# QizhiPei/FABind

Measured on AMD Instinct MI355X. Metric: complexes/sec fwd+bwd (1500p/40l nodes), full IaBNet on the whole graph (pocket model + 4-layer complex model + distance-map head on all nodes / pairs) with the pocket-cls + pocket-centre + coord + distmap + distmap-by-coords + distill losses (BASELINE configs[2] read literally), higher is better.
Workload: dtype bf16

## Files before the change

### fabind_amd/_lib.py

```python
import ctypes
import os

import torch

from . import config as _cfg

_HERE = os.path.dirname(os.path.abspath(__file__))
LIB_PATH = _cfg.knob("FABIND_LIB") or os.path.join(_HERE, "libfabind_hip.so")

ABI_VERSION = 19
DT_F32, DT_BF16 = 0, 1
ACT_NONE, ACT_SILU, ACT_RELU, ACT_SIGMOID, ACT_STORED_DERIV = 0, 1, 2, 3, 4
GEMM_FAM_NT_F32, GEMM_FAM_NT_F32_BF16, GEMM_FAM_NT_BF16, GEMM_FAM_GLDS, GEMM_FAM_PIPE, GEMM_FAM_X3, GEMM_FAM_X3_PRO, GEMM_FAM_PERSIST = range(8)

LNR_8S16, LNR_8S32, LNR_V8_1, LNR_V8_2, LNR_V8_3, LNR_V8_4, LNR_S2, LNR_S8, LNR_S16, LNR_S32, LNR_COUNT = range(11)
LNB_8S16, LNB_8S32, LNB_V8_1, LNB_V8_2, LNB_V8_3, LNB_S2, LNB_S8, LNB_S16, LNB_S20, LNB_S32, LNB_COUNT = range(11)
RST_BF16_1, RST_BF16_2, RST_BF16_4, RST_GENERIC, RST_COUNT = range(5)
ELF_WAVE1, ELF_WAVE1_TAIL, ELF_WAVE2_TAIL, ELF_CHUNK, ELF_COUNT = range(5)
ELB_NPL1, ELB_NPL2, ELB_NPL3, ELB_COUNT = range(4)

_vp, _i, _f, _l = ctypes.c_void_p, ctypes.c_int, ctypes.c_float, ctypes.c_long


class GemmArgs(ctypes.Structure):
# ... 58 lines not shown
    "fabind_gcl_edge_fused_bwd_set_tile": [_i],
    "fabind_gcl_edge_fused_bwd_tile": [],
    "fabind_gcl_edge_fused_bwd_set_variant": [_i],
    "fabind_gcl_edge_fused_set_variant": [_i],
    "fabind_gcl_edge_fused_variant": [],
    "fabind_gcl_edge_fused_bwd_variant": [],
    "fabind_gcl_edge_fused_bwd_variant_for": [_i],
    "fabind_row_stats": [_vp, _i, _i, _f, _i, _i, _vp, _vp, _vp],
    "fabind_layernorm_rows": [_vp, _i, _i, _vp, _vp, _f, _i, _i, _vp, _i, _i, _i, _vp],
    "fabind_edge_ln_concat": [_vp, _i, _i, _vp, _vp, _vp, _vp, _vp, _f, _i, _vp, _i, _i, _i, _vp],
    "fabind_edge_lnfold": [_vp, _i, _i, _i, _vp, _vp, _vp, _vp, _f, _vp, _vp, _vp, _vp, _i, _vp, _f, ctypes.c_uint, _vp],
    "fabind_edge_lnfold_bwd_blocks": [_i],
    "fabind_edge_lnfold_bwd": [_vp, _i, _i, _i, _vp, _vp, _vp, _vp, _f, _vp, _vp, _vp, _vp, _vp, _i, _f, _vp, _vp, _vp, _vp, _i, _vp],
    "fabind_layernorm_rows_form": [_vp, _i, _i, _vp, _i, _i],
    "fabind_layernorm_rows_bwd_form": [_vp, _i, _vp, _i, _vp, _i, _i],
    "fabind_row_stats_form": [_vp, _i, _i, _i],
    "fabind_edge_lnfold_form": [_i, _i, ctypes.POINTER(_i)],
    "fabind_edge_lnfold_blocks": [_i],
    "fabind_edge_lnfold_bwd_form": [_i, ctypes.POINTER(_i)],
    "fabind_inter_coord_fold_blocks": [_i],
    "fabind_inter_coord_fold": [_vp, _i, _i, _vp, _vp, _vp, _f, _f, _vp, _vp, _vp, _i, _vp, _f, ctypes.c_uint, _vp],
    "fabind_post_optimize": [_vp, _vp, _vp, _vp, _vp, _i, _i, _i, _i, _f, _vp, _vp, _vp, _vp],
    "fabind_distmap_generate": [_vp, _vp, _vp, _vp, _vp, _vp, _vp, _vp, _vp, _vp, _i, _i, _i, _i, _i, _i, _l, _i, _i, _i, _i,
                                _vp, _vp, _vp, _vp, _vp, _vp, _vp, _vp],
    "fabind_sym_automorphisms": [_vp, _vp, _vp, _vp, _i, _i, _i, _vp, _vp, _vp, _vp, _vp, _vp],
    "fabind_sym_score": [_vp, _i, _i, _vp, _vp, _vp, _vp, _vp, _i, _i, _vp, _vp, _vp, _vp, _vp, _vp],
    "fabind_pose_stats": [_vp, _vp, _vp, _i, _vp, _vp, _vp],
    "fabind_rank_loss_fwd": [_vp, _vp, _vp, _i, _i, _i, _vp, _vp, _vp, _vp],
    "fabind_multi_copy": [_vp, _i, _i, _vp],
    "fabind_adam_chunk": [],
    "fabind_multi_sqnorm": [_vp, _i, _i, _vp, _vp, _vp, _vp],
    "fabind_multi_adam": [_vp, _i, _i, _vp, _vp, _vp, _f, _i, _vp, _vp, _vp],
    "fabind_zero_empty_rows": [_vp, _i, _vp, _i, _i, _i, _vp, _i, _i, _vp],
    "fabind_split_sum": [_vp, _i, ctypes.c_long, _vp, _i, ctypes.c_long, _vp, _vp],
    "fabind_segment_sum": [_vp, _i, _i, _i, _vp, _vp, _i, _i, _i, _vp, _i, _vp, _i, _vp],
    "fabind_coord_update": [_vp, _vp, _vp, _i, _vp, _vp, _i, _i, _f, _vp, _vp, _vp],
    "fabind_cross_attn_fwd": [_vp, _i, _vp, _vp, _i, _vp, _i, _vp, _i, _i, _i, _vp, _i, _i, _f, _vp, _i, _vp, _i, _vp, _i,
                              _vp],
    "fabind_cross_attn_mfma_fwd": [_vp, _i, _vp, _vp, _i, _vp, _i, _vp, _i, _i, _i, _vp, _i, _i, _f, _vp, _i, _vp, _i, _vp, _i,
                                   _vp],
    "fabind_cross_attn_fused_fwd": [_vp, _i, _vp, _vp, _i, _vp, _i, _vp, _i, _vp, _vp, _vp, _vp, _i, _i, _i, _i, _i, _f, _vp, _i, _vp, _i, _vp, _vp],
    "fabind_cross_attn_fused_bwd": [ctypes.POINTER(AttnFusedBwdArgs), _i, _i, _i, _i, _i, _i, _vp],
    "fabind_pair_bot_pack": [_vp, _i, _vp, _i, _vp, _vp, _vp, _vp, _i, _vp, _i, _l, _vp],
    "fabind_pair_bo_pack": [_vp, _i, _vp, _i, _vp, _vp, _vp, _vp, _i, _vp, _i, _l, _vp],
    "fabind_cross_attn_mfma_bwd": [_vp, _i, _vp, _i, _vp, _i, _i, _i, _vp, _i, _i, _i, _f, _vp, _vp, _vp, _vp, _vp, _vp, _vp,
                                   _vp, _vp, _vp],
    "fabind_pair_bmat": [_vp, _i, _vp, _i, _i, _vp, _i, _vp, _i, _vp],
    "fabind_pair_hadamard": [_vp, _vp, _i, _i, _vp, _vp, _i, _i, _vp, _vp, _i, _vp, _i, _i, _vp],
    "fabind_inter_attn_fwd": [_vp, _i, _vp, _i, _i, _vp, _i, _vp, _vp, _vp, _vp, _vp, _vp, _vp, _i, _vp, _vp, _vp,
                              _vp, _f, _i, _vp, _vp, _vp, _vp, _vp, _vp, _vp],
    "fabind_inter_attn_fwd_rows": [_vp, _i, _vp, _i, _i, _vp, _i, _vp, _vp, _vp, _vp, _vp, _vp, _vp, _i, _vp, _vp, _vp,
                                   _vp, _f, _i, _vp, _vp, _vp, _vp, _vp, _vp, _vp, _i, _i, _vp],
    "fabind_layernorm_rows_bwd": [_vp, _i, _i, _vp, _vp, _i, _i, _f, _i, _i, _vp, _i, _i, _vp, _vp, _i, _vp],
    "fabind_edge_concat": [_vp, _i, _i, _vp, _vp, _vp, _i, _vp, _i, _i, _i, _vp],
    "fabind_las_step": [_vp, _vp, _vp, _vp, _vp, _vp, _vp, _i, _i, _f, _f, _vp, _vp, _vp],
    "fabind_select_rows": [_vp, _vp, _vp, _i, _i, _vp, _vp],
    "fabind_add": [_vp, _vp, _vp, _l, _vp],
    "fabind_mul_dact": [_vp, _i, _vp, _i, _i, _vp, _i, _l, _f, _vp],
    "fabind_mul_dact_colsum": [_vp, _i, _vp, _i, _i, _vp, _i, _i, _i, _vp, _vp, _i, _f, _vp],
    "fabind_drop_mix": [_vp, _vp, _vp, _l, _f, ctypes.c_uint, _vp],
    "fabind_drop_mix_bwd": [_vp, _vp, _vp, _l, _f, ctypes.c_uint, _vp],
    "fabind_mul_dropmask_colsum": [_vp, _i, _vp, _i, _i, _i, _f, ctypes.c_uint, _vp, _vp, _i, _vp],
    "fabind_rowdot_bwd": [_vp, _i, _vp, _i, _vp, _i, _i, _i, _vp, _vp, _vp, _i, _vp],
    "fabind_edge_geom_bwd": [_vp, _vp, _vp, _vp, _vp, _vp, _vp, _vp, _vp, _vp, _i, _i, _i, _vp, _vp, _vp, _vp],
    "fabind_gcl_pre_bwd": [_vp, _i, _i, _vp, _vp, _i, _vp, _vp, _vp, _i, _vp],
    "fabind_gather_dact": [_vp, _i, _vp, _vp, _i, _i, _vp, _i, _i, _i, _vp],
    "fabind_coord_update_bwd": [_vp, _vp, _vp, _i, _i, _f, _vp, _vp, _vp, _vp],
    "fabind_cross_attn_bwd": [_vp, _i, _vp, _i, _vp, _i, _i, _i, _vp, _i, _i, _i, _f, _vp, _vp, _vp, _vp, _vp, _vp, _vp,
                              _vp, _vp, _vp],
    "fabind_pair_bias_cat": [_vp, _i, _vp, _i, _i, _i, _vp, _i, _vp, _i, _vp, _vp, _i, _vp, _i, _vp, _vp],
    "fabind_batched_transpose_pad": [_vp, _i, _vp, _i, _i, _i, _i, _vp, _vp],
    "fabind_node_chain_fwd": [_vp, _i, _vp, _i, _vp, _vp, _vp, _vp, _vp, _vp, _i, _i, _vp, _i, _vp, _i, _vp, _i, _i, _i, _vp],
    "fabind_node_chain_x3_fwd": [_vp, _i, _vp, _i, _vp, _vp, _vp, _vp, _vp, _vp, _vp, _vp, _vp, _vp, _i, _i, _vp, _i, _vp, _i, _vp, _i, _vp, _i, _vp, _i,
                                 _i, _i, _vp],
    "fabind_rows_hadamard_bwd": [_vp, _i, _i, _vp, _i, _i, _vp, _vp, _vp, _i, _vp, _i, _vp],
    "fabind_pair_hadamard_bwd_grid": [_vp, _i, _i, _vp, _i, _i, _vp, _vp, _vp, _vp, _i, _vp, _i, _vp],
    "fabind_pair_hadamard_bwd_rows": [_vp, _i, _i, _vp, _i, _i, _vp, _i, _i, _vp, _vp, _vp, _vp, _i, _vp, _i, _vp, _i, _vp],
    "fabind_pair_hadamard_bwd": [_vp, _i, _i, _vp, _vp, _i, _i, _vp, _vp, _i, _i, _vp, _vp, _i, _vp, _vp, _i, _vp, _vp, _i,
                                 _vp],
    "fabind_inter_attn_bwd": [_vp, _i, _vp, _i, _i, _vp, _vp, _vp, _vp, _vp, _vp, _vp, _vp, _vp, _vp, _vp, _vp, _f, _i,
                              _vp, _vp, _vp, _vp, _vp, _vp, _vp, _vp, _vp, _vp, _i, _vp],
    "fabind_inter_attn_bwd_rows": [_vp, _i, _vp, _i, _i, _vp, _vp, _vp, _vp, _vp, _vp, _vp, _vp, _vp, _vp, _vp, _vp, _f, _i,
                                   _vp, _vp, _vp, _vp, _vp, _vp, _vp, _vp, _vp, _vp, _i, _vp, _i, _i, _vp],
    "fabind_las_step_bwd": [_vp, _vp, _vp, _vp, _vp, _vp, _vp, _vp, _i, _i, _f, _f, _vp, _vp, _vp],
    "fabind_pair_bias_bwd": [_vp, _i, _vp, _i, _i, _vp, _vp, _i, _i, _i, _vp, _vp, _vp, _vp, _vp],
    "fabind_pair_bias_btcat": [_vp, _i, _vp, _vp, _vp, _i, _i, _i, _vp, _i, _i, _vp],
    "fabind_pair_bias_finish": [_vp, _vp, _i, _i, _vp, _vp, _i, _vp, _vp, _l, _vp],
    "fabind_pack_frag_multi": [_vp, _vp, _i, _vp],
    "fabind_lower_bound": [_vp, _i, _vp, _i, _vp, _vp],
    "fabind_pocket_center_fwd": [_vp, _vp, _vp, _vp, _i, _i, _f, _i, _vp, _vp, _vp],
    "fabind_pocket_center_bwd": [_vp, _vp, _vp, _vp, _i, _i, _f, _vp, _vp, _vp, _vp, _vp],
    "fabind_pair_dist_fwd": [_vp, _i, _i, _vp, _vp, _f, _f, _f, _vp, _vp],
    "fabind_pair_dist_bwd": [_vp, _i, _i, _vp, _vp, _vp, _f, _f, _f, _vp, _vp, _vp],
    "fabind_block_hadamard_fwd": [_vp, _i, _i, _vp, _i, _vp, _i, _i, _vp, _i, _vp],
    "fabind_block_hadamard_bwd": [_vp, _i, _i, _vp, _i, _vp, _i, _vp, _i, _i, _vp, _i, _i, _vp, _vp, _i, _vp, _i, _vp],
    "fabind_loss_fwd": [_vp, _vp, _l, _vp, _vp, _vp, _l, _vp, _vp, _i, _vp, _l, _vp, _vp, _l, _f, _f, _f, _f, _f, _f, _vp, _vp, _vp, _vp, _vp, _vp],
    "fabind_loss_bwd": [_vp, _vp, _l, _vp, _vp, _vp, _l, _vp, _vp, _i, _l, _vp, _vp, _l, _f, _f, _f, _f, _f, _f, _vp, _vp, _vp,
                        _vp, _vp, _vp, _vp, _vp, _vp],
    "fabind_layernorm_fwd": [_vp, _vp, _vp, _f, _i, _i, _vp, _vp, _vp, _vp],
    "fabind_layernorm_bwd": [_vp, _vp, _vp, _vp, _vp, _i, _i, _vp, _vp, _vp, _vp],
}

_lib = None


def load():
    global _lib
    if _lib is not None:
        return _lib
    if not os.path.exists(LIB_PATH):
        raise RuntimeError(
            "fabind_amd: %s is missing -- build it with `python -m fabind_amd.build` (hipcc, gfx950). "
            "There is no CPU/eager fallback for the hot path." % LIB_PATH)
    lib = ctypes.CDLL(LIB_PATH)
    lib.fabind_last_error.restype = ctypes.c_char_p
    lib.fabind_abi_version.restype = ctypes.c_int
    got = lib.fabind_abi_version()
    if got != ABI_VERSION:
        raise RuntimeError("fabind_amd: %s has ABI version %d, this binding needs %d -- rebuild with `python -m fabind_amd.build`"
                           % (LIB_PATH, got, ABI_VERSION))
    lib.fabind_sizeof_args.argtypes, lib.fabind_sizeof_args.restype = [ctypes.c_int], ctypes.c_int
    lib.fabind_cross_attn_bwd_scratch.argtypes, lib.fabind_cross_attn_bwd_scratch.restype = [_i, _i, _i], ctypes.c_long
    lib.fabind_pair_bias_cat_parts.argtypes, lib.fabind_pair_bias_cat_parts.restype = [_i, _i], ctypes.c_long
    lib.fabind_cross_attn_fused_bwd_scratch.argtypes, lib.fabind_cross_attn_fused_bwd_scratch.restype = [_i, _i, _i, _i, _i], ctypes.c_long
    lib.fabind_cross_attn_fused_bwd_parts.argtypes, lib.fabind_cross_attn_fused_bwd_parts.restype = [_i, _i], ctypes.c_int
    lib.fabind_pair_bias_finish_parts.argtypes, lib.fabind_pair_bias_finish_parts.restype = [_i], ctypes.c_int
    lib.fabind_loss_blocks.argtypes, lib.fabind_loss_blocks.restype = [_l, _l, _l], ctypes.c_int
    for nm in ("fabind_pair_block_tile", "fabind_pair_block_chunk"):
        getattr(lib, nm).argtypes, getattr(lib, nm).restype = [], ctypes.c_int
    for which, mirror in enumerate((GemmArgs, EdgeBwdArgs, PairUpdateArgs, TnJob, AttnFusedBwdArgs, AdamRow)):
        if lib.fabind_sizeof_args(which) != ctypes.sizeof(mirror):
            raise RuntimeError("fabind_amd: ctypes mirror %s is %d bytes, the library's struct is %d -- _lib.py and "
                               "include/fabind_hip.h disagree" % (mirror.__name__, ctypes.sizeof(mirror),
                                                                  lib.fabind_sizeof_args(which)))
    for nm in ("fabind_gemm_set_config", "fabind_gemm_set_persistent", "fabind_gemm_set_small_m", "fabind_gemm_set_x3_tile", "fabind_gemm_tn_set_waves",
               "fabind_gemm_tn_set_exp", "fabind_gcl_edge_fused_set_xcd_aware", "fabind_gcl_edge_fused_bwd3_set_exp",
               "fabind_gcl_edge_fused_bwd4_set_exp"):
        getattr(lib, nm).argtypes, getattr(lib, nm).restype = [ctypes.c_int], None
    lib.fabind_gemm_tn_tile_n.argtypes, lib.fabind_gemm_tn_tile_n.restype = [], ctypes.c_int
    for name, argt in SIGNATURES.items():
        fn = getattr(lib, name)
        fn.argtypes = argt
        fn.restype = ctypes.c_int
    for k in _cfg.KNOBS.values():
        if k.category == "native-dev" and _cfg.knob(k.name) is not None:
            getattr(lib, k.setter)(_cfg.knob(k.name))
    _lib = lib
    return lib


_DEBUG_SYNC = _cfg.knob("FABIND_DEBUG_SYNC")


def check(rc, what):
    if rc != 0:
        raise RuntimeError("%s failed (rc=%d): %s" % (what, rc, load().fabind_last_error().decode()))
    if _DEBUG_SYNC:
        print("[fabind] " + what, flush=True)
        torch.cuda.synchronize()


def ptr(t):
    if t is None:
        return None
    if not t.is_cuda:
        raise RuntimeError("fabind_amd kernels need HIP device tensors; got a %s tensor" % t.device)
# ... 20 lines not shown
```

### fabind_amd/csrc/gcl.hip

```cpp
#include "common.h"
#include "fabind_hip.h"

__global__ __launch_bounds__(256) void gcl_pre_kernel(const void* __restrict__ AB, int ab_dt, int ldab, int H,
                                                      const int* row, const int* col, const float* rhohat,
                                                      const float* __restrict__ w_r, void* pre, int pre_dt, int E, int act,
                                                      void* dact_out) {
    const int lane = threadIdx.x & 63;
    int e = blockIdx.x * 4 + (threadIdx.x >> 6);
    if (e >= E) return;
    const size_t a = (size_t)row[e] * ldab, b = (size_t)col[e] * ldab + H;
    const float rh = rhohat[e];
    for (int c = lane * 4; c < H; c += 256) {
        float4 va = ld4_any(AB, ab_dt, a + c), vb = ld4_any(AB, ab_dt, b + c), w = *(const float4*)(w_r + c);
        const float4 z = make_float4(va.x + vb.x + rh * w.x, va.y + vb.y + rh * w.y, va.z + vb.z + rh * w.z,
                                     va.w + vb.w + rh * w.w);
        st4_any(pre, pre_dt, (size_t)e * H + c,
                make_float4(apply_act(z.x, act), apply_act(z.y, act), apply_act(z.z, act), apply_act(z.w, act)));
        if (dact_out)
            st4_any(dact_out, pre_dt, (size_t)e * H + c,
                    make_float4(apply_dact(z.x, act), apply_dact(z.y, act), apply_dact(z.z, act), apply_dact(z.w, act)));
    }
}

#define GP_PASSES 4
// ... 79 lines not shown
                      (!dact_out || (uintptr_t)dact_out % 16 == 0) && ((uintptr_t)w_r % 16 == 0);
#define GP_LAUNCH4(LPE_, A16_, O16_, D_)                                                                             \
    hipLaunchKernelGGL((gcl_pre8_kernel<LPE_, A16_, O16_, D_>),                                                      \
                       dim3((E + 4 * (64 / LPE_) * GP_PASSES - 1) / (4 * (64 / LPE_) * GP_PASSES)), dim3(256), 0, stream, \
                       AB, ldab, row, col, rhohat, w_r, pre, E, act, dact_out)
#define GP_LAUNCH(LPE_)                                                                                              \
    do {                                                                                                             \
        const bool a16 = ab_dt == FB_DT_BF16, o16 = pre_dt == FB_DT_BF16;                                            \
        if (a16 && o16 && dact_out) GP_LAUNCH4(LPE_, true, true, true);                                              \
        else if (a16 && o16) GP_LAUNCH4(LPE_, true, true, false);                                                    \
        else if (!a16 && o16 && dact_out) GP_LAUNCH4(LPE_, false, true, true);                                       \
        else if (!a16 && o16) GP_LAUNCH4(LPE_, false, true, false);                                                  \
        else if (!a16 && !o16 && dact_out) GP_LAUNCH4(LPE_, false, false, true);                                     \
        else if (!a16 && !o16) GP_LAUNCH4(LPE_, false, false, false);                                                \
        else if (dact_out) GP_LAUNCH4(LPE_, true, false, true);                                                      \
        else GP_LAUNCH4(LPE_, true, false, false);                                                                   \
    } while (0)
    if (vec8 && H == 512) GP_LAUNCH(64);
    else if (vec8 && H == 256) GP_LAUNCH(32);
    else if (vec8 && H == 128) GP_LAUNCH(16);
    else if (vec8 && H == 64) GP_LAUNCH(8);
    else
        hipLaunchKernelGGL(gcl_pre_kernel, dim3((E + 3) / 4), dim3(256), 0, stream, AB, ab_dt, ldab, H, row, col, rhohat,
                           w_r, pre, pre_dt, E, act, dact_out);
#undef GP_LAUNCH
#undef GP_LAUNCH4
    FB_CHECK_LAUNCH();
    return 0;
}


template <int NSLAB, int U>
__device__ __forceinline__ void ss_accum(const void* __restrict__ Z, int z_dt, int ldz, int H, const int* eidx, int act,
                                         int lane, int e0, int e1, int estep, F8 (&acc)[NSLAB]) {
    int ee = e0;
    for (; ee + (U - 1) * estep < e1; ee += U * estep) {
        int e[U];
#pragma unroll
        for (int u = 0; u < U; ++u) e[u] = eidx ? eidx[ee + u * estep] : ee + u * estep;
#pragma unroll
        for (int s = 0; s < NSLAB; ++s) {
            const int c = s * 512 + lane * 8;
            if (c < H) {
                F8 v[U];
#pragma unroll
                for (int u = 0; u < U; ++u) v[u] = ld8_any(Z, z_dt, (size_t)e[u] * ldz + c);
#pragma unroll
                for (int u = 0; u < U; ++u)
#pragma unroll
                    for (int k = 0; k < 8; ++k) acc[s].v[k] += apply_act(v[u].v[k], act);
            }
        }
    }
    if (ee < e1) {
        int e[U];
        bool ok[U];
#pragma unroll
        for (int u = 0; u < U; ++u) {
            ok[u] = ee + u * estep < e1;
            e[u] = ok[u] ? (eidx ? eidx[ee + u * estep] : ee + u * estep) : 0;
        }
#pragma unroll
        for (int s = 0; s < NSLAB; ++s) {
            const int c = s * 512 + lane * 8;
            if (c < H) {
                F8 v[U];
#pragma unroll
                for (int u = 0; u < U; ++u) {
                    if (ok[u]) v[u] = ld8_any(Z, z_dt, (size_t)e[u] * ldz + c);
                    else
#pragma unroll
                        for (int k = 0; k < 8; ++k) v[u].v[k] = 0.f;
                }
#pragma unroll
                for (int u = 0; u < U; ++u)
#pragma unroll
                    for (int k = 0; k < 8; ++k) acc[s].v[k] += apply_act(v[u].v[k], act);
            }
        }
    }
}

template <int NSLAB>
__global__ __launch_bounds__(256) void segment_sum_kernel(const void* __restrict__ Z, int z_dt, int ldz, int H,
                                                          const int* rowptr, const int* eidx, int act, float* out,
                                                          int ldo, int n_rows, bf16_t* out16, int ldo16, int heavy_min) {
    const int lane = threadIdx.x & 63;
    const int r = blockIdx.x * 4 + (threadIdx.x >> 6);
    if (r >= n_rows) return;
    const int e0 = rowptr[r], e1 = rowptr[r + 1];
    if (e1 - e0 > heavy_min) return;
    F8 acc[NSLAB];
#pragma unroll
    for (int s = 0; s < NSLAB; ++s)
#pragma unroll
        for (int k = 0; k < 8; ++k) acc[s].v[k] = 0.f;
    ss_accum<NSLAB, 8 / NSLAB>(Z, z_dt, ldz, H, eidx, act, lane, e0, e1, 1, acc);
#pragma unroll
    for (int s = 0; s < NSLAB; ++s) {
        const int c = s * 512 + lane * 8;
        if (c < H) {
            if (out) {
                float* o = out + (size_t)r * ldo + c;
                *(float4*)o = make_float4(acc[s].v[0], acc[s].v[1], acc[s].v[2], acc[s].v[3]);
                *(float4*)(o + 4) = make_float4(acc[s].v[4], acc[s].v[5], acc[s].v[6], acc[s].v[7]);
            }
            if (out16) st8_any(out16, FB_DT_BF16, (size_t)r * ldo16 + c, acc[s]);
        }
    }
}

template <int NSLAB>
__global__ __launch_bounds__(1024) void segment_sum_heavy_kernel(const void* __restrict__ Z, int z_dt, int ldz, int H,
                                                                 const int* rowptr, const int* eidx, int act, float* out,
                                                                 int ldo, int n_rows, bf16_t* out16, int ldo16, int rpw, int heavy_min) {
    __shared__ F8 part[15][NSLAB * 64];
    __shared__ int heavy[1024];
    __shared__ int n_heavy;
    const int lane = threadIdx.x & 63, w = threadIdx.x >> 6;
    if (threadIdx.x == 0) n_heavy = 0;
    __syncthreads();
    const int rr = blockIdx.x * rpw + threadIdx.x;
    if ((int)threadIdx.x < rpw && rr < n_rows && rowptr[rr + 1] - rowptr[rr] > heavy_min) heavy[atomicAdd(&n_heavy, 1)] = rr;
    __syncthreads();
    const int nh = n_heavy;
    for (int q = 0; q < nh; ++q) {
        const int r = heavy[q];
        F8 acc[NSLAB];
#pragma unroll
        for (int s = 0; s < NSLAB; ++s)
#pragma unroll
            for (int k = 0; k < 8; ++k) acc[s].v[k] = 0.f;
        ss_accum<NSLAB, 8 / NSLAB>(Z, z_dt, ldz, H, eidx, act, lane, rowptr[r] + w, rowptr[r + 1], 16, acc);
        if (w > 0) {
#pragma unroll
            for (int s = 0; s < NSLAB; ++s) part[w - 1][s * 64 + lane] = acc[s];
        }
        __syncthreads();
        if (w == 0) {
#pragma unroll
            for (int s = 0; s < NSLAB; ++s) {
                for (int k = 0; k < 15; ++k) {
                    const F8 p = part[k][s * 64 + lane];
#pragma unroll
                    for (int t = 0; t < 8; ++t) acc[s].v[t] += p.v[t];
                }
                const int c = s * 512 + lane * 8;
                if (c < H) {
                    if (out) {
                        float* o = out + (size_t)r * ldo + c;
                        *(float4*)o = make_float4(acc[s].v[0], acc[s].v[1], acc[s].v[2], acc[s].v[3]);
                        *(float4*)(o + 4) = make_float4(acc[s].v[4], acc[s].v[5], acc[s].v[6], acc[s].v[7]);
                    }
                    if (out16) st8_any(out16, FB_DT_BF16, (size_t)r * ldo16 + c, acc[s]);
                }
            }
        }
        __syncthreads();
    }
}

extern "C" int fabind_segment_sum(const void* Z, int z_dt, int ldz, int H, const int* rowptr, const int* eidx,
                                  int n_rows, int n_edges, int act, float* out, int ldo, void* out16v, int ldo16,
                                  hipStream_t stream) {
    bf16_t* out16 = (bf16_t*)out16v;
    FB_REQUIRE(H % 8 == 0 && ldz % 8 == 0 && ldo % 4 == 0, "fabind_segment_sum: H/ldz must be multiples of 8, ldo of 4");
    FB_REQUIRE(H <= 1024, "fabind_segment_sum: H <= 1024");
    FB_REQUIRE(out != nullptr || out16 != nullptr, "fabind_segment_sum: no output");
    FB_REQUIRE(((uintptr_t)Z % 16 == 0) && ((uintptr_t)out % 16 == 0), "fabind_segment_sum: 16-byte alignment");
    FB_REQUIRE(out16 == nullptr || (ldo16 % 8 == 0 && (uintptr_t)out16 % 16 == 0), "fabind_segment_sum: out16 needs 16-byte alignment and ldo16 % 8 == 0");
    if (n_rows <= 0) return 0;
    (void)n_edges;
    int rpw = 1024;
    while (rpw > 64 && (n_rows + rpw - 1) / rpw < 256) rpw >>= 1;
    const int heavy_min = n_rows < 16384 ? 32 : 128;
    const dim3 g((n_rows + 3) / 4), gh((n_rows + rpw - 1) / rpw);
    if (H <= 512) {
        hipLaunchKernelGGL((segment_sum_kernel<1>), g, dim3(256), 0, stream, Z, z_dt, ldz, H, rowptr, eidx, act, out, ldo, n_rows, out16, ldo16, heavy_min);
        hipLaunchKernelGGL((segment_sum_heavy_kernel<1>), gh, dim3(1024), 0, stream, Z, z_dt, ldz, H, rowptr, eidx, act, out, ldo, n_rows, out16, ldo16, rpw, heavy_min);
    } else {
        hipLaunchKernelGGL((segment_sum_kernel<2>), g, dim3(256), 0, stream, Z, z_dt, ldz, H, rowptr, eidx, act, out, ldo, n_rows, out16, ldo16, heavy_min);
        hipLaunchKernelGGL((segment_sum_heavy_kernel<2>), gh, dim3(1024), 0, stream, Z, z_dt, ldz, H, rowptr, eidx, act, out, ldo, n_rows, out16, ldo16, rpw, heavy_min);
    }
    FB_CHECK_LAUNCH();
    return 0;
}

__global__ __launch_bounds__(256) void coord_update_kernel(const float* __restrict__ x, const float* __restrict__ d,
                                                           const float* __restrict__ s_part, int n_part,
                                                           const float* weight, const int* rowptr, int n_rows, int mean,
                                                           float clampv, float* x_out, float* s_out) {
    const int lane = threadIdx.x & 63;
    int r = blockIdx.x * 4 + (threadIdx.x >> 6);
    if (r >= n_rows) return;
    const int e0 = rowptr[r], e1 = rowptr[r + 1];
    float ax = 0.f, ay = 0.f, az = 0.f;
    for (int e = e0 + lane; e < e1; e += 64) {
        float s = 0.f;
        for (int k = 0; k < n_part; ++k) s += s_part[(size_t)e * n_part + k];
        if (weight) s *= weight[e];
        if (s_out) s_out[e] = s;
        ax += d[(size_t)e * 3] * s; ay += d[(size_t)e * 3 + 1] * s; az += d[(size_t)e * 3 + 2] * s;
    }
    ax = wave_sum(ax); ay = wave_sum(ay); az = wave_sum(az);
    if (lane == 0) {
        const int deg = e1 - e0;
        const float den = mean ? (float)(deg < 1 ? 1 : deg) : 1.f;
        float tx = ax / den, ty = ay / den, tz = az / den;
        tx = fminf(fmaxf(tx, -clampv), clampv); ty = fminf(fmaxf(ty, -clampv), clampv); tz = fminf(fmaxf(tz, -clampv), clampv);
        x_out[(size_t)r * 3] = x[(size_t)r * 3] + tx;
        x_out[(size_t)r * 3 + 1] = x[(size_t)r * 3 + 1] + ty;
        x_out[(size_t)r * 3 + 2] = x[(size_t)r * 3 + 2] + tz;
    }
}

extern "C" int fabind_coord_update(const float* x, const float* d, const float* s_part, int n_part,
                                   const float* weight, const int* rowptr, int n_rows, int mean, float clampv,
                                   float* x_out, float* s_out, hipStream_t stream) {
    if (n_rows <= 0) return 0;
    hipLaunchKernelGGL(coord_update_kernel, dim3((n_rows + 3) / 4), dim3(256), 0, stream, x, d, s_part, n_part, weight,
                       rowptr, n_rows, mean, clampv, x_out, s_out);
    FB_CHECK_LAUNCH();
    return 0;
}

__global__ __launch_bounds__(256) void zero_empty_rows_kernel(const int* __restrict__ rowptr, int n_rows, void* out, int out_dt, int ld,
                                                              int C, void* out2, int out2_dt, int ld2) {
    const int lane = threadIdx.x & 63;
    const int r = blockIdx.x * 4 + (threadIdx.x >> 6);
    if (r >= n_rows || rowptr[r] != rowptr[r + 1]) return;
    for (int c = lane; c < C; c += 64) {
        st_any(out, out_dt, (size_t)r * ld + c, 0.f);
        if (out2) st_any(out2, out2_dt, (size_t)r * ld2 + c, 0.f);
    }
}

extern "C" int fabind_zero_empty_rows(const int* rowptr, int n_rows, void* out, int out_dt, int ld, int C, void* out2, int out2_dt,
                                      int ld2, hipStream_t stream) {
    if (n_rows <= 0 || C <= 0) return 0;
    FB_REQUIRE(rowptr != nullptr && out != nullptr, "fabind_zero_empty_rows: rowptr / out");
    hipLaunchKernelGGL(zero_empty_rows_kernel, dim3((n_rows + 3) / 4), dim3(256), 0, stream, rowptr, n_rows, out, out_dt, ld, C, out2,
                       out2_dt, ld2);
    FB_CHECK_LAUNCH();
    return 0;
}


__global__ __launch_bounds__(256) void pack_frag_multi_kernel(const FabindPackSeg* __restrict__ segs) {
    const FabindPackSeg sg = segs[blockIdx.y];
    const int N = sg.N, Kd = sg.K;
    const long n_vec = (long)N * Kd / 8;
    bf16_t* dst = (bf16_t*)sg.dst;
    for (long t = (long)blockIdx.x * 256 + threadIdx.x; t < n_vec; t += (long)gridDim.x * 256) {
        const int r = (int)(t & 15), q = (int)((t >> 4) & 3);
        const long tb = t >> 6;
        const int nb = (int)(tb % (N / 16)), kb = (int)(tb / (N / 16));
        const long n = (long)nb * 16 + r, k0 = (long)kb * 32 + q * 8;
        uint32_t w[4];
#pragma unroll
        for (int j = 0; j < 4; ++j) {
            float a, b;
            const long i0 = n * sg.src_sr + (k0 + 2 * j) * sg.src_sc, i1 = i0 + sg.src_sc;
            if (sg.src_dt == FB_DT_BF16) {
                a = bf16_to_f32(((const bf16_t*)sg.src)[i0]);
                b = bf16_to_f32(((const bf16_t*)sg.src)[i1]);
            } else {
// ... 30 lines not shown
```

### fabind_amd/csrc/inter_attn_rows.hip

```cpp
#include "common.h"
#include "fabind_hip.h"

#define IA_HEAVY 8

template <int NS>
__global__ __launch_bounds__(256) void inter_attn_fwd_rows_kernel(
    const float* __restrict__ qkv, int ldqkv, const float* __restrict__ cv, int ldcv, int H, const float* __restrict__ h,
    int ldh, const float* __restrict__ x, const float* __restrict__ d, const float* __restrict__ rhohat,
    const int* rowptr, const int* col, const int* red_idx, const float* bias_red, int bias_np,
    const float* __restrict__ w_rk, const float* __restrict__ w_rv, const float* __restrict__ wcr,
    const float* __restrict__ w3, float clampv, int n_rows, float* h_out, float* x_out, float* alpha, float* cvs, bf16_t* h16,
    const float* __restrict__ s_ext, const int* __restrict__ order, int n_heavy, int n_act) {
    __shared__ float4 sAcc[4][NS * 64];
    __shared__ float sSc[4][8];
    const int lane = threadIdx.x & 63, wv = threadIdx.x >> 6;
    const bool coop = (int)blockIdx.x < n_heavy;
    const int idx = coop ? (int)blockIdx.x : n_heavy + ((int)blockIdx.x - n_heavy) * 4 + wv;
    if (idx >= n_rows) return;
    const int r = order[idx];
    if (idx >= n_act) {
#pragma unroll
        for (int s = 0; s < NS; ++s) {
            const int c = s * 256 + lane * 4;
            if (c < H) {
// ... 98 lines not shown
        for (int s = 0; s < NS; ++s) {
            const int c = s * 256 + lane * 4;
            if (c < H) {
                const float4 hv = *(const float4*)(h + (size_t)r * ldh + c);
                const float4 wvv = *(const float4*)(w_rv + c);
                const float4 o = make_float4(hv.x + (acc[s].x + sar * wvv.x) * inv, hv.y + (acc[s].y + sar * wvv.y) * inv,
                                             hv.z + (acc[s].z + sar * wvv.z) * inv, hv.w + (acc[s].w + sar * wvv.w) * inv);
                *(float4*)(h_out + (size_t)r * ldh + c) = o;
                if (h16) *(uint2*)(h16 + (size_t)r * H + c) = make_uint2(pack2_bf16(o.x, o.y), pack2_bf16(o.z, o.w));
            }
        }
        if (lane == 0) {
            const float tx = fminf(fmaxf(ax * inv, -clampv), clampv), ty = fminf(fmaxf(ay * inv, -clampv), clampv),
                        tz = fminf(fmaxf(az * inv, -clampv), clampv);
            x_out[(size_t)r * 3] = x[(size_t)r * 3] + tx;
            x_out[(size_t)r * 3 + 1] = x[(size_t)r * 3 + 1] + ty;
            x_out[(size_t)r * 3 + 2] = x[(size_t)r * 3 + 2] + tz;
        }
    } else {
#pragma unroll
        for (int s = 0; s < NS; ++s) sAcc[wv][s * 64 + lane] = acc[s];
        if (lane == 0) { sSc[wv][0] = m; sSc[wv][1] = l; sSc[wv][2] = sar; sSc[wv][3] = ax; sSc[wv][4] = ay; sSc[wv][5] = az; }
        __syncthreads();
        const float M = fmaxf(fmaxf(sSc[0][0], sSc[1][0]), fmaxf(sSc[2][0], sSc[3][0]));
        float f[4], L = 0.f, SAR = 0.f, AX = 0.f, AY = 0.f, AZ = 0.f;
#pragma unroll
        for (int w = 0; w < 4; ++w) {
            f[w] = sSc[w][1] > 0.f ? __expf(sSc[w][0] - M) : 0.f;
            L += f[w] * sSc[w][1]; SAR += f[w] * sSc[w][2]; AX += f[w] * sSc[w][3]; AY += f[w] * sSc[w][4]; AZ += f[w] * sSc[w][5];
        }
        inv = 1.f / L;
        for (int g = threadIdx.x; g < NS * 64; g += 256) {
            const int c = (g >> 6) * 256 + (g & 63) * 4;
            if (c < H) {
                float4 a = make_float4(0.f, 0.f, 0.f, 0.f);
#pragma unroll
                for (int w = 0; w < 4; ++w) {
                    const float4 p = sAcc[w][g];
                    a.x += f[w] * p.x; a.y += f[w] * p.y; a.z += f[w] * p.z; a.w += f[w] * p.w;
                }
                const float4 hv = *(const float4*)(h + (size_t)r * ldh + c);
                const float4 wvv = *(const float4*)(w_rv + c);
                const float4 o = make_float4(hv.x + (a.x + SAR * wvv.x) * inv, hv.y + (a.y + SAR * wvv.y) * inv,
                                             hv.z + (a.z + SAR * wvv.z) * inv, hv.w + (a.w + SAR * wvv.w) * inv);
                *(float4*)(h_out + (size_t)r * ldh + c) = o;
                if (h16) *(uint2*)(h16 + (size_t)r * H + c) = make_uint2(pack2_bf16(o.x, o.y), pack2_bf16(o.z, o.w));
            }
        }
        if (threadIdx.x == 0) {
            const float tx = fminf(fmaxf(AX * inv, -clampv), clampv), ty = fminf(fmaxf(AY * inv, -clampv), clampv),
                        tz = fminf(fmaxf(AZ * inv, -clampv), clampv);
            x_out[(size_t)r * 3] = x[(size_t)r * 3] + tx;
            x_out[(size_t)r * 3 + 1] = x[(size_t)r * 3 + 1] + ty;
            x_out[(size_t)r * 3 + 2] = x[(size_t)r * 3 + 2] + tz;
        }
        m = M;
    }
    __builtin_amdgcn_fence(__ATOMIC_RELEASE, "wavefront");
    __builtin_amdgcn_fence(__ATOMIC_ACQUIRE, "wavefront");
    for (int e = ws + lane; e < we; e += 64) alpha[e] = __expf(alpha[e] - m) * inv;
}

extern "C" int fabind_inter_attn_fwd_rows(const float* qkv, int ldqkv, const float* cv, int ldcv, int H, const float* h,
                                          int ldh, const float* x, const float* d, const float* rhohat, const int* rowptr,
                                          const int* col, const int* red_idx, const float* bias_red, int bias_np,
                                          const float* w_rk, const float* w_rv, const float* wcr, const float* w3,
                                          float clampv, int n_rows, float* h_out, float* x_out, float* alpha, float* cvs,
                                          const float* s_ext, void* h16, const int* order, int n_heavy, int n_act, hipStream_t stream) {
    FB_REQUIRE(H % 4 == 0 && ldqkv % 4 == 0 && ldcv % 4 == 0 && ldh % 4 == 0, "fabind_inter_attn_fwd_rows: % 4");
    FB_REQUIRE(H <= 1024, "fabind_inter_attn_fwd_rows: H <= 1024");
    FB_REQUIRE(order != nullptr && 0 <= n_heavy && n_heavy <= n_act && n_act <= n_rows, "fabind_inter_attn_fwd_rows: order / counts");
    if (n_rows <= 0) return 0;
    dim3 grid(n_heavy + (n_rows - n_heavy + 3) / 4), block(256);
#define LAUNCH(NS)                                                                                                   \
    hipLaunchKernelGGL((inter_attn_fwd_rows_kernel<NS>), grid, block, 0, stream, qkv, ldqkv, cv, ldcv, H, h, ldh, x, d, \
                       rhohat, rowptr, col, red_idx, bias_red, bias_np, w_rk, w_rv, wcr, w3, clampv, n_rows, h_out, \
                       x_out, alpha, cvs, (bf16_t*)h16, s_ext, order, n_heavy, n_act)
    if (H <= 256) LAUNCH(1); else if (H <= 512) LAUNCH(2); else LAUNCH(4);
#undef LAUNCH
    FB_CHECK_LAUNCH();
    return 0;
}

template <int NS>
__global__ __launch_bounds__(256) void inter_attn_bwd_a_rows_kernel(
    const float* __restrict__ qkv, int ldqkv, const float* __restrict__ cv, int ldcv, int H, const float* __restrict__ d,
    const float* __restrict__ rhohat, const int* rowptr, const int* col, const float* __restrict__ w_rk,
    const float* __restrict__ w_rv, const float* __restrict__ wcr, const float* __restrict__ w3, const float* alpha,
    const float* cvs, float clampv, int n_rows, const float* __restrict__ dh_out, const float* __restrict__ dx_out,
    float* dqkv, float* dd, float* drh, float* dlogit, float* dcp, float* wpart, const int* __restrict__ order, int n_heavy, int n_act) {
    extern __shared__ float4 shp[];
    float (*sS)[4] = (float (*)[4])(shp + 4 * NS * 64);
    const int lane = threadIdx.x & 63, wv = threadIdx.x >> 6;
    const float4 z4 = make_float4(0.f, 0.f, 0.f, 0.f);
    float4 a_wrk[NS], a_wrv[NS], a_wcr[NS], a_w3[NS], wk[NS], wvv[NS], wc[NS], w3v[NS];
#pragma unroll
    for (int s = 0; s < NS; ++s) {
        const int c = s * 256 + lane * 4;
        a_wrk[s] = z4; a_wrv[s] = z4; a_wcr[s] = z4; a_w3[s] = z4; wk[s] = z4; wvv[s] = z4; wc[s] = z4; w3v[s] = z4;
        if (c < H) {
            wk[s] = *(const float4*)(w_rk + c); wvv[s] = *(const float4*)(w_rv + c);
            wc[s] = *(const float4*)(wcr + c); w3v[s] = *(const float4*)(w3 + c);
        }
    }
    const int n_hturns = (n_heavy + (int)gridDim.x - 1) / (int)gridDim.x;
    const int n_lturns = (n_rows - n_heavy + (int)gridDim.x * 4 - 1) / ((int)gridDim.x * 4);
    for (int turn = 0; turn < n_hturns + n_lturns; ++turn) {
        const bool coop = turn < n_hturns;
        int idx;
        if (coop) idx = turn * (int)gridDim.x + (int)blockIdx.x;
        else idx = n_heavy + ((turn - n_hturns) * (int)gridDim.x + (int)blockIdx.x) * 4 + wv;
        if (coop ? idx >= n_heavy : idx >= n_rows) continue;
        const int r = order[idx];
        if (idx >= n_act) {
#pragma unroll
            for (int s = 0; s < NS; ++s) {
                const int c = s * 256 + lane * 4;
                if (c < H) *(float4*)(dqkv + (size_t)r * ldqkv + c) = z4;
            }
            continue;
        }
        const int e0 = rowptr[r], e1 = rowptr[r + 1];
        int ws = e0, we = e1;
        if (coop) {
            const int per = (e1 - e0 + 3) >> 2;
            ws = min(e1, e0 + wv * per);
            we = min(e1, ws + per);
        }
        float4 qv[NS], gh[NS], dq[NS];
        float qw = 0.f, gwv = 0.f;
#pragma unroll
        for (int s = 0; s < NS; ++s) {
            const int c = s * 256 + lane * 4;
            qv[s] = z4; gh[s] = z4; dq[s] = z4;
            if (c < H) {
                qv[s] = *(const float4*)(qkv + (size_t)r * ldqkv + c);
                gh[s] = *(const float4*)(dh_out + (size_t)r * H + c);
                qw += qv[s].x * wk[s].x + qv[s].y * wk[s].y + qv[s].z * wk[s].z + qv[s].w * wk[s].w;
                gwv += gh[s].x * wvv[s].x + gh[s].y * wvv[s].y + gh[s].z * wvv[s].z + gh[s].w * wvv[s].w;
            }
        }
        qw = wave_sum(qw); gwv = wave_sum(gwv);
        float tx = 0.f, ty = 0.f, tz = 0.f;
        for (int e = e0 + lane; e < e1; e += 64) {
            const float w = alpha[e] * cvs[e];
            tx += w * d[(size_t)e * 3]; ty += w * d[(size_t)e * 3 + 1]; tz += w * d[(size_t)e * 3 + 2];
        }
        tx = wave_sum(tx); ty = wave_sum(ty); tz = wave_sum(tz);
        const float gx = fabsf(tx) <= clampv ? dx_out[(size_t)r * 3] : 0.f;
        const float gy = fabsf(ty) <= clampv ? dx_out[(size_t)r * 3 + 1] : 0.f;
        const float gz = fabsf(tz) <= clampv ? dx_out[(size_t)r * 3 + 2] : 0.f;
        float S = 0.f;
        float4 pa[NS], pb[NS];
        auto fetch_v = [&](int cn) {
#pragma unroll
            for (int s = 0; s < NS; ++s) {
                const int c = s * 256 + lane * 4;
                pa[s] = z4;
                if (c < H) pa[s] = *(const float4*)(qkv + (size_t)cn * ldqkv + 2 * H + c);
            }
        };
        for (int eb = ws; eb < we; eb += 64) {
            const int ne = min(64, we - eb);
            int my_col = 0;
            float my_rh = 0.f, my_al = 0.f, my_cvs = 0.f, my_gd = 0.f, my_da = 0.f;
            if (lane < ne) {
                const int e = eb + lane;
                my_col = col[e]; my_rh = rhohat[e]; my_al = alpha[e]; my_cvs = cvs[e];
                my_gd = gx * d[(size_t)e * 3] + gy * d[(size_t)e * 3 + 1] + gz * d[(size_t)e * 3 + 2];
            }
            fetch_v(__shfl(my_col, 0, 64));
            for (int j = 0; j < ne; ++j) {
                const float rh = __shfl(my_rh, j, 64);
                float hp = 0.f;
                float4 vv[NS];
#pragma unroll
                for (int s = 0; s < NS; ++s) vv[s] = pa[s];
                if (j + 1 < ne) fetch_v(__shfl(my_col, j + 1, 64));
#pragma unroll
                for (int s = 0; s < NS; ++s)
                    hp += gh[s].x * vv[s].x + gh[s].y * vv[s].y + gh[s].z * vv[s].z + gh[s].w * vv[s].w;
                hp = wave_sum(hp) + rh * gwv;
                const float da = hp + __shfl(my_cvs, j, 64) * __shfl(my_gd, j, 64);
                S += __shfl(my_al, j, 64) * da;
                if (lane == j) my_da = da;
            }
            if (lane < ne) dlogit[eb + lane] = my_da;
        }
        if (coop) {
            if (lane == 0) sS[wv][0] = S;
            __syncthreads();
            S = ((sS[0][0] + sS[1][0]) + sS[2][0]) + sS[3][0];
        }
        __builtin_amdgcn_fence(__ATOMIC_RELEASE, "wavefront");
        __builtin_amdgcn_fence(__ATOMIC_ACQUIRE, "wavefront");
        float s_lrh = 0.f, s_arh = 0.f;
        auto fetch_kc = [&](int cn) {
#pragma unroll
            for (int s = 0; s < NS; ++s) {
                const int c = s * 256 + lane * 4;
                pa[s] = z4; pb[s] = z4;
                if (c < H) {
                    pa[s] = *(const float4*)(qkv + (size_t)cn * ldqkv + H + c);
                    pb[s] = *(const float4*)(cv + (size_t)cn * ldcv + c);
                }
            }
        };
        for (int eb = ws; eb < we; eb += 64) {
            const int ne = min(64, we - eb);
            int my_col = 0;
            float my_rh = 0.f, my_al = 0.f, my_cvs = 0.f, my_gd = 0.f, my_da = 0.f, o_dl = 0.f, o_dc = 0.f, o_drh = 0.f;
            if (lane < ne) {
                const int e = eb + lane;
                my_col = col[e]; my_rh = rhohat[e]; my_al = alpha[e]; my_cvs = cvs[e]; my_da = dlogit[e];
                my_gd = gx * d[(size_t)e * 3] + gy * d[(size_t)e * 3 + 1] + gz * d[(size_t)e * 3 + 2];
            }
            fetch_kc(__shfl(my_col, 0, 64));
            for (int j = 0; j < ne; ++j) {
                const float rh = __shfl(my_rh, j, 64), al = __shfl(my_al, j, 64);
                float4 kks[NS], ccs[NS];
#pragma unroll
                for (int s = 0; s < NS; ++s) { kks[s] = pa[s]; ccs[s] = pb[s]; }
                if (j + 1 < ne) fetch_kc(__shfl(my_col, j + 1, 64));
                const float dl = al * (__shfl(my_da, j, 64) - S);
                const float dc = al * __shfl(my_gd, j, 64);
                float dsum = 0.f;
#pragma unroll
                for (int s = 0; s < NS; ++s) {
                    const int c = s * 256 + lane * 4;
                    if (c < H) {
                        const float4 kk = kks[s], cc = ccs[s];
                        dq[s].x += dl * (kk.x + rh * wk[s].x); dq[s].y += dl * (kk.y + rh * wk[s].y);
                        dq[s].z += dl * (kk.z + rh * wk[s].z); dq[s].w += dl * (kk.w + rh * wk[s].w);
                        const float ux = cc.x + rh * wc[s].x, uy = cc.y + rh * wc[s].y, uz = cc.z + rh * wc[s].z, uw = cc.w + rh * wc[s].w;
                        const float px = w3v[s].x * dsilu_f(ux), py = w3v[s].y * dsilu_f(uy), pz = w3v[s].z * dsilu_f(uz), pw = w3v[s].w * dsilu_f(uw);
                        dsum += px * wc[s].x + py * wc[s].y + pz * wc[s].z + pw * wc[s].w;
                        a_wcr[s].x += dc * rh * px; a_wcr[s].y += dc * rh * py; a_wcr[s].z += dc * rh * pz; a_wcr[s].w += dc * rh * pw;
                        a_w3[s].x += dc * silu_f(ux); a_w3[s].y += dc * silu_f(uy); a_w3[s].z += dc * silu_f(uz); a_w3[s].w += dc * silu_f(uw);
                    }
                }
                dsum = wave_sum(dsum);
                s_lrh += dl * rh; s_arh += al * rh;
                if (lane == j) { o_dl = dl; o_dc = dc; o_drh = dl * qw + al * gwv + dc * dsum; }
            }
            if (lane < ne) {
                const int e = eb + lane;
                dlogit[e] = o_dl;
                dcp[e] = o_dc;
                drh[e] = o_drh;
                const float w = my_al * my_cvs;
                dd[(size_t)e * 3] = w * gx; dd[(size_t)e * 3 + 1] = w * gy; dd[(size_t)e * 3 + 2] = w * gz;
            }
        }
        if (!coop) {
#pragma unroll
            for (int s = 0; s < NS; ++s) {
                const int c = s * 256 + lane * 4;
                if (c < H) {
                    *(float4*)(dqkv + (size_t)r * ldqkv + c) = dq[s];
                    a_wrk[s].x += s_lrh * qv[s].x; a_wrk[s].y += s_lrh * qv[s].y; a_wrk[s].z += s_lrh * qv[s].z; a_wrk[s].w += s_lrh * qv[s].w;
                    a_wrv[s].x += s_arh * gh[s].x; a_wrv[s].y += s_arh * gh[s].y; a_wrv[s].z += s_arh * gh[s].z; a_wrv[s].w += s_arh * gh[s].w;
                }
            }
        } else {
#pragma unroll
            for (int s = 0; s < NS; ++s) shp[wv * NS * 64 + s * 64 + lane] = dq[s];
            if (lane == 0) { sS[wv][1] = s_lrh; sS[wv][2] = s_arh; }
            __syncthreads();
            for (int g = threadIdx.x; g < NS * 64; g += 256) {
                const int c = (g >> 6) * 256 + (g & 63) * 4;
                if (c < H) {
                    float4 t = shp[g];
#pragma unroll
                    for (int w = 1; w < 4; ++w) {
                        const float4 o = shp[w * NS * 64 + g];
                        t.x += o.x; t.y += o.y; t.z += o.z; t.w += o.w;
                    }
                    *(float4*)(dqkv + (size_t)r * ldqkv + c) = t;
                }
            }
            if (wv == 0) {
                const float tl = ((sS[0][1] + sS[1][1]) + sS[2][1]) + sS[3][1], ta = ((sS[0][2] + sS[1][2]) + sS[2][2]) + sS[3][2];
#pragma unroll
                for (int s = 0; s < NS; ++s) {
                    a_wrk[s].x += tl * qv[s].x; a_wrk[s].y += tl * qv[s].y; a_wrk[s].z += tl * qv[s].z; a_wrk[s].w += tl * qv[s].w;
                    a_wrv[s].x += ta * gh[s].x; a_wrv[s].y += ta * gh[s].y; a_wrv[s].z += ta * gh[s].z; a_wrv[s].w += ta * gh[s].w;
                }
            }
            __syncthreads();
        }
    }
    __syncthreads();
#pragma unroll
    for (int s = 0; s < NS; ++s) {
        shp[(0 * 4 + wv) * NS * 64 + s * 64 + lane] = a_wrk[s];
        shp[(1 * 4 + wv) * NS * 64 + s * 64 + lane] = a_wrv[s];
        shp[(2 * 4 + wv) * NS * 64 + s * 64 + lane] = a_wcr[s];
        shp[(3 * 4 + wv) * NS * 64 + s * 64 + lane] = a_w3[s];
    }
    __syncthreads();
    for (int i2 = threadIdx.x; i2 < 4 * NS * 64; i2 += 256) {
        const int qn = i2 / (NS * 64), rem = i2 % (NS * 64);
        const int c = (rem / 64) * 256 + (rem % 64) * 4;
        if (c >= H) continue;
        float4 t = shp[(qn * 4 + 0) * NS * 64 + rem];
#pragma unroll
        for (int w2 = 1; w2 < 4; ++w2) {
            const float4 o = shp[(qn * 4 + w2) * NS * 64 + rem];
            t.x += o.x; t.y += o.y; t.z += o.z; t.w += o.w;
        }
        *(float4*)(wpart + ((size_t)blockIdx.x * 4 + qn) * H + c) = t;
    }
}

template <int NS>
__global__ __launch_bounds__(256) void inter_attn_bwd_b_rows_kernel(
    const float* __restrict__ qkv, int ldqkv, const float* __restrict__ cv, int ldcv, int H, const float* rhohat,
    const int* rowptr, const int* col, const int* mirror, const int* red_idx, const float* __restrict__ wcr,
    const float* __restrict__ w3, const float* alpha, const float* dlogit, const float* dcp, int n_rows,
    const float* __restrict__ dh_out, float* dqkv, float* dcv, float* dbias_red, const int* __restrict__ order, int n_heavy, int n_act) {
    extern __shared__ float4 shb[];
    const int lane = threadIdx.x & 63, wv = threadIdx.x >> 6;
    const bool coop = (int)blockIdx.x < n_heavy;
    const int idx = coop ? (int)blockIdx.x : n_heavy + ((int)blockIdx.x - n_heavy) * 4 + wv;
    if (idx >= n_rows) return;
    const int n = order[idx];
    const float4 z4 = make_float4(0.f, 0.f, 0.f, 0.f);
    float4 dk[NS], dv[NS], dc[NS], cvn[NS], wc[NS], w3v[NS];
#pragma unroll
    for (int s = 0; s < NS; ++s) {
        const int c = s * 256 + lane * 4;
        dk[s] = z4; dv[s] = z4; dc[s] = z4; cvn[s] = z4; wc[s] = z4; w3v[s] = z4;
        if (c < H && idx < n_act) {
            cvn[s] = *(const float4*)(cv + (size_t)n * ldcv + c);
            wc[s] = *(const float4*)(wcr + c); w3v[s] = *(const float4*)(w3 + c);
        }
    }
    if (idx < n_act) {
        const int e0 = rowptr[n], e1 = rowptr[n + 1];
        int ws = e0, we = e1;
        if (coop) {
            const int per = (e1 - e0 + 3) >> 2;
            ws = min(e1, e0 + wv * per);
            we = min(e1, ws + per);
        }
        for (int eb = ws; eb < we; eb += 64) {
            const int ne = min(64, we - eb);
            int m_l = 0;
            float dl_l = 0.f, al_l = 0.f, dcm_l = 0.f, rh_l = 0.f;
            if (lane < ne) {
                const int e = eb + lane, me = mirror[e];
                m_l = col[e];
                dl_l = dlogit[me]; al_l = alpha[me]; dcm_l = dcp[me]; rh_l = rhohat[me];
                if (n < m_l) dbias_red[red_idx[e]] = dlogit[e] + dl_l;
            }
#pragma unroll 2
            for (int j = 0; j < ne; ++j) {
                const int m = __shfl(m_l, j, 64);
                const float dl = __shfl(dl_l, j, 64), al = __shfl(al_l, j, 64), dcm = __shfl(dcm_l, j, 64), rh = __shfl(rh_l, j, 64);
#pragma unroll
                for (int s = 0; s < NS; ++s) {
                    const int c = s * 256 + lane * 4;
                    if (c < H) {
                        const float4 qm = *(const float4*)(qkv + (size_t)m * ldqkv + c);
                        const float4 gm = *(const float4*)(dh_out + (size_t)m * H + c);
                        dk[s].x += dl * qm.x; dk[s].y += dl * qm.y; dk[s].z += dl * qm.z; dk[s].w += dl * qm.w;
                        dv[s].x += al * gm.x; dv[s].y += al * gm.y; dv[s].z += al * gm.z; dv[s].w += al * gm.w;
                        dc[s].x += dcm * w3v[s].x * dsilu_f(cvn[s].x + rh * wc[s].x);
                        dc[s].y += dcm * w3v[s].y * dsilu_f(cvn[s].y + rh * wc[s].y);
                        dc[s].z += dcm * w3v[s].z * dsilu_f(cvn[s].z + rh * wc[s].z);
                        dc[s].w += dcm * w3v[s].w * dsilu_f(cvn[s].w + rh * wc[s].w);
                    }
                }
            }
        }
    }
    if (!coop) {
#pragma unroll
        for (int s = 0; s < NS; ++s) {
            const int c = s * 256 + lane * 4;
            if (c < H) {
                *(float4*)(dqkv + (size_t)n * ldqkv + H + c) = dk[s];
                *(float4*)(dqkv + (size_t)n * ldqkv + 2 * H + c) = dv[s];
                *(float4*)(dcv + (size_t)n * ldcv + c) = dc[s];
            }
        }
        return;
    }
#pragma unroll
    for (int s = 0; s < NS; ++s) {
        shb[(0 * 4 + wv) * NS * 64 + s * 64 + lane] = dk[s];
        shb[(1 * 4 + wv) * NS * 64 + s * 64 + lane] = dv[s];
        shb[(2 * 4 + wv) * NS * 64 + s * 64 + lane] = dc[s];
    }
    __syncthreads();
    for (int i2 = threadIdx.x; i2 < 3 * NS * 64; i2 += 256) {
        const int qn = i2 / (NS * 64), g = i2 % (NS * 64);
        const int c = (g >> 6) * 256 + (g & 63) * 4;
        if (c >= H) continue;
        float4 t = shb[(qn * 4 + 0) * NS * 64 + g];
#pragma unroll
        for (int w = 1; w < 4; ++w) {
            const float4 o = shb[(qn * 4 + w) * NS * 64 + g];
            t.x += o.x; t.y += o.y; t.z += o.z; t.w += o.w;
        }
        if (qn == 0) *(float4*)(dqkv + (size_t)n * ldqkv + H + c) = t;
        else if (qn == 1) *(float4*)(dqkv + (size_t)n * ldqkv + 2 * H + c) = t;
        else *(float4*)(dcv + (size_t)n * ldcv + c) = t;
    }
}

extern "C" int fabind_inter_attn_bwd_rows(const float* qkv, int ldqkv, const float* cv, int ldcv, int H, const float* d,
                                          const float* rhohat, const int* rowptr, const int* col, const int* mirror,
                                          const int* red_idx, const float* w_rk, const float* w_rv, const float* wcr,
                                          const float* w3, const float* alpha, const float* cvs, float clampv, int n_rows,
                                          const float* dh_out, const float* dx_out, float* dqkv, float* dcv, float* dd,
                                          float* drh, float* dbias_red, float* dlogit, float* dcp, float* wpart, int nblk,
                                          const int* order, int n_heavy, int n_act, hipStream_t stream) {
    if (n_rows <= 0) return 0;
    FB_REQUIRE(H % 4 == 0 && H <= 1024, "fabind_inter_attn_bwd_rows: H % 4, H <= 1024");
    FB_REQUIRE(order != nullptr && 0 <= n_heavy && n_heavy <= n_act && n_act <= n_rows && nblk > 0, "fabind_inter_attn_bwd_rows: order / counts");
    dim3 gb(n_heavy + (n_rows - n_heavy + 3) / 4);
#define LA(NS) do {                                                                                                    \
        size_t lds = (size_t)16 * NS * 64 * sizeof(float4);                                                            \
        hipLaunchKernelGGL((inter_attn_bwd_a_rows_kernel<NS>), dim3(nblk), dim3(256), lds, stream, qkv, ldqkv, cv, ldcv, H, d, \
                           rhohat, rowptr, col, w_rk, w_rv, wcr, w3, alpha, cvs, clampv, n_rows, dh_out, dx_out, dqkv, dd, \
                           drh, dlogit, dcp, wpart, order, n_heavy, n_act);                                             \
        size_t ldsb = (size_t)12 * NS * 64 * sizeof(float4);                                                           \
        hipLaunchKernelGGL((inter_attn_bwd_b_rows_kernel<NS>), gb, dim3(256), ldsb, stream, qkv, ldqkv, cv, ldcv, H, rhohat, rowptr, \
                           col, mirror, red_idx, wcr, w3, alpha, dlogit, dcp, n_rows, dh_out, dqkv, dcv, dbias_red, order,  \
                           n_heavy, n_act);                                                                            \
    } while (0)
    if (H <= 256) LA(1); else if (H <= 512) LA(2); else LA(4);
#undef LA
    FB_CHECK_LAUNCH();
    return 0;
}
```

### fabind_amd/engine.py

```python
import math

import numpy as np
import torch

from . import config as _cfg
from . import kernels as K
from . import ops

from .config import fp32_storage, get_precision, set_precision, split_sites
from .config import x3_backward_bf16 as config_x3_backward_bf16
from .param_pack import EagerPack, ParamPack


FUSED_EDGE = True
LAYOUT_CACHE = _cfg.knob("FABIND_LAYOUT_CACHE")
DEBUG_GRAPH = _cfg.knob("FABIND_DEBUG_GRAPH")
DEBUG_CAPTURE = None


def _wd():
    return torch.float32 if fp32_storage() else torch.bfloat16


def _count(idx, n):
# ... 479 lines not shown
    x_new = ops.coord_update(x, d, s, g.rp_ctx, mean=True, clampv=clampv)
    t = ops.linear(hin, p["Wn1"], p["bn1"], x2=agg, act_epi=K.ACT_SILU, out_dtype=ad)
    if pdrop > 0.0:
        h_new = h + _drop(ops.linear(t, p["Wn2"], p["bn2"]), pdrop)
    else:
        h_new = ops.linear(t, p["Wn2"], p["bn2"], residual=h)
    return h_new, x_new


def cross_attention(p, h, lay, pairbias, layer, pdrop=0.0):
    fast = _fast(h, p["Wo_p"])
    od = ops.act_dtype()
    c16 = (lambda t: _b16(t)) if fast else (lambda t: t)
    h = ops.shared_grad(h)
    hc = ops.take_rows(h, lay.c_index64)
    scale = 1.0 / math.sqrt(32.0)
    nograd = fast or (get_precision() == "bf16x3" and not ops.needs_grad(h, p["Wo_p"], getattr(pairbias, "a0b0", None)))
    fused = nograd and isinstance(pairbias, ops.PairBias) and pairbias.can_fuse() and not pairbias.has_tensors()
    ftrain = (not fast) and pdrop >= 0.0 and isinstance(pairbias, ops.PairBias) and not pairbias.has_tensors() and pairbias.can_fuse_train() \
        and ops.needs_grad(h, p["Wo_p"], pairbias.a0b0)
    if not fused and not ftrain:
        pbt = pairbias.tensors() if isinstance(pairbias, ops.PairBias) else pairbias
        bias_p, bias_c = pbt[2 * layer], pbt[2 * layer + 1]
    qg = ops.linear(c16(h), p["Wqg_p"], p["bqg_p"])
    kv = ops.linear(hc if p.get("Wkv_p32") is not None else c16(hc), p["Wkv_p"], W32=p.get("Wkv_p32"))
    og = ops.cross_attn_fused(qg, kv, pairbias, 2 * layer, 0, lay, scale) if fused else \
        ops.cross_attn_fused_train(qg, kv, pairbias, 2 * layer, 0, scale) if ftrain else \
        ops.cross_attn(qg, kv, bias_p, 0, 4, lay.desc_pf, lay.B, lay.max_P, lay.max_C, scale)
    hp = ops.linear(og if p.get("Wo_p32") is not None else c16(og), p["Wo_p"], p["bo_p"], residual=h, want16=True, W32=p.get("Wo_p32"),
                    p_drop=pdrop)
    hp = ops.shared_grad(hp)
    hp16 = c16(hp)
    qg = ops.linear(c16(hc), p["Wqg_c"], p["bqg_c"])
    kv = ops.linear(hp if p.get("Wkv_c32") is not None else hp16, p["Wkv_c"], W32=p.get("Wkv_c32"))
    og = ops.cross_attn_fused(qg, kv, pairbias, 2 * layer + 1, 1, lay, scale) if fused else \
        ops.cross_attn_fused_train(qg, kv, pairbias, 2 * layer + 1, 1, scale) if ftrain else \
        ops.cross_attn(qg, kv, bias_c, 0, 4, lay.desc_cf, lay.B, lay.max_C, lay.max_P, scale)
    hc = ops.linear(og if p.get("Wo_c32") is not None else c16(og), p["Wo_c"], p["bo_c"], residual=hc, p_drop=pdrop, W32=p.get("Wo_c32"))
    if fast:
        hp2 = None
        if p.get("Wt_p32") is not None:
            hp2 = _node_chain_x3(p, "_ncx_tp", p["Wt_p32"], p["bt1_p"], p["bt2_p"], K.ACT_RELU, 1, hp, None, hp, True)
            if hp2 is None:
                hp2 = ops.mlp2(hp, p["Wt1_p"], p["bt1_p"], K.ACT_RELU, p["Wt2_p"], p["bt2_p"], residual=hp, want16=True, W32=p["Wt_p32"])
        else:
            hp2 = _node_chain(p, "_nc_tp", p["Wt1_p"], p["bt1_p"], p["Wt2_p"], p["bt2_p"], K.ACT_RELU, 1, hp16, None, hp, True)
        if hp2 is None:
            t = ops.linear(hp16, p["Wt1_p"], p["bt1_p"], act_epi=K.ACT_RELU, out_dtype=od)
            hp2 = ops.linear(t, p["Wt2_p"], p["bt2_p"], residual=hp, want16=True)
        hp = hp2
        hc16 = c16(hc)
        if p.get("Wt_c32") is not None:
            hc2 = _node_chain_x3(p, "_ncx_tc", p["Wt_c32"], p["bt1_c"], p["bt2_c"], K.ACT_RELU, 1, hc, None, hc, False)
            if hc2 is None:
                hc2 = ops.mlp2(hc, p["Wt1_c"], p["bt1_c"], K.ACT_RELU, p["Wt2_c"], p["bt2_c"], residual=hc, W32=p["Wt_c32"])
        else:
            hc2 = _node_chain(p, "_nc_tc", p["Wt1_c"], p["bt1_c"], p["Wt2_c"], p["bt2_c"], K.ACT_RELU, 1, hc16, None, hc, False)
        if hc2 is None:
            t = ops.linear(hc16, p["Wt1_c"], p["bt1_c"], act_epi=K.ACT_RELU, out_dtype=od)
            hc2 = ops.linear(t, p["Wt2_c"], p["bt2_c"], residual=hc)
        hc = hc2
    elif (get_precision() == "bf16x3" and p["Wt1_p"].dtype == torch.float32
          and not ops.needs_grad(hp, hc, p["Wt1_p"], p["Wt2_p"], p["Wt1_c"], p["Wt2_c"])):
        hp2 = _node_chain_x3(p, "_ncx3_tp", (p["Wt1_p"], p["Wt2_p"]), p["bt1_p"], p["bt2_p"], K.ACT_RELU, 1, hp, None, hp, True)
        hp = hp2 if hp2 is not None else ops.mlp2(hp, p["Wt1_p"], p["bt1_p"], K.ACT_RELU, p["Wt2_p"], p["bt2_p"], residual=hp, want16=True)
        hc2 = _node_chain_x3(p, "_ncx3_tc", (p["Wt1_c"], p["Wt2_c"]), p["bt1_c"], p["bt2_c"], K.ACT_RELU, 1, hc, None, hc, False)
        hc = hc2 if hc2 is not None else ops.mlp2(hc, p["Wt1_c"], p["bt1_c"], K.ACT_RELU, p["Wt2_c"], p["bt2_c"], residual=hc)
    else:
        hp = ops.mlp2(hp, p["Wt1_p"], p["bt1_p"], K.ACT_RELU, p["Wt2_p"], p["bt2_p"], residual=hp, want16=True, W32=p.get("Wt_p32"),
                      chain=p.get("_ncx_tp"))
        hc = ops.mlp2(hc, p["Wt1_c"], p["bt1_c"], K.ACT_RELU, p["Wt2_c"], p["bt2_c"], residual=hc, W32=p.get("Wt_c32"), chain=p.get("_ncx_tc"))
    return ops.put_rows(hp, hc, lay.c_index64)


def att_layer(p, h, x, lay, g, a0b0, pairbias, layer, clampv, pdrop=0.0, pdrop_row=0.0):
    H = h.shape[1]
    h = cross_attention(p, h, lay, pairbias, layer, pdrop_row)
    if pdrop == 0.0:
        h = ops.shared_grad(h)
    h16 = _b16(h) if _fast(h, x, p["Wqkv"]) else h
    ab32 = ops.linear(h16, p["W_ab32"], p["b_ab32"])
    hd = ops.pair_hadamard(a0b0, H, ab32, 64, g.red_p, g.red_c, graph=g)
    bias_part = ops.linear_rowdot(hd, p["Wcomp1"], p["bcomp1"], p["u"], act_epi=K.ACT_RELU)
    qkv = ops.linear(h if p.get("Wqkv32") is not None else h16, p["Wqkv"], p["bqkv"], want16=True, W32=p.get("Wqkv32"))
    d, rhohat = ops.edge_geom(x, g.row_int, g.col_int, g.rp_int, lay, g.int_by_col)
    h_new, x_new, alpha = ops.inter_attn(qkv, None, H, h, x, d, rhohat, g, bias_part, p["w_rk"], p["w_rv"], p["wcr"],
                                         p["w3"], clampv, Wc=p["Wc"], bc=p["bc"], own_h=(pdrop == 0.0), Wc32=p.get("Wc32"))
    if pdrop > 0.0:
        h_new = ops.drop_mix(h, h_new, pdrop)
    return h_new, x_new, alpha


def egnn_forward(P, h, x, lay, g, las, x_las, a0b0, pairbias, scale, step, drop=None):
    clampv = 10.0 / scale
    dp = drop or {}
    h = ops.linear(h, P["W_in"], P["b_in"], want16=True, W32=P.get("W_in32"), p_drop=dp.get("gnn", 0.0))
    cap = DEBUG_CAPTURE
    for i in range(P["L"]):
        h, x = gcl_layer(P["gcl"][i], h, x, lay, g, clampv, dp.get("gcl", 0.0))
        if cap is not None:
            cap["gcl_%d.h" % i], cap["gcl_%d.x" % i] = h.detach().clone(), x.detach().clone()
        h, x, alpha = att_layer(P["att"][i], h, x, lay, g, a0b0, pairbias, i, clampv, dp.get("att", 0.0), dp.get("row", 0.0))
        if cap is not None:
            cap["att_%d.h" % i], cap["att_%d.x" % i], cap["att_%d.alpha" % i] = h.detach().clone(), x.detach().clone(), alpha.detach().clone()
        x = ops.las_step(x, x_las, las, lay, step, 15.0 / scale)
        if cap is not None:
            cap["las_%d.xout" % i] = x.detach().clone()
    h, x = gcl_layer(P["out_layer"], h, x, lay, g, clampv, dp.get("out", 0.0))
    return ops.linear(_drop(h, dp.get("gnn", 0.0)), P["W_out"], P["b_out"]), x


def pair_bias_all(P, a0b0, lay):
    H = P["H"]
    return ops.PairBias(a0b0, H, P["pb_wcomp"], P["pb_bconst"], lay)


_PREFETCHED = []


def _record_streams(obj, stream_):
    for v in vars(obj).values():
        for t in (v if isinstance(v, (tuple, list)) else (v,)):
            if torch.is_tensor(t) and t.is_cuda:
                t.record_stream(stream_)


def prefetch(model, X, batch_id, segment_id, compound_edge_index):
    import weakref
    lay = Layout(batch_id, segment_id)
    ex = model.extract_edges
    brow = compound_edge_index[0].to(torch.int32).contiguous()
    bcol = compound_edge_index[1].to(torch.int32).contiguous()
    g = Graph(lay, X.detach().reshape(-1, 3).float().contiguous(), brow, bcol, lay.ranges(brow), float(ex.intra_cutoff),
              float(ex.inter_cutoff))
    g._prefetched_bonds = (brow, bcol)
    ev = torch.cuda.Event()
    ev.record(torch.cuda.current_stream(X.device))
    _PREFETCHED[:] = [e for e in _PREFETCHED if e[0]() is not None and e[2]() is not None]
    _PREFETCHED.insert(0, (weakref.ref(X), X._version, weakref.ref(batch_id), lay, g, ev))
    del _PREFETCHED[4:]
    return lay, g


def _take_prefetched(X, batch_id):
    for i, (wx, ver, wb, lay, g, ev) in enumerate(_PREFETCHED):
        if wx() is X and wb() is batch_id and ver == X._version:
            del _PREFETCHED[i]
            cur = torch.cuda.current_stream(X.device)
            cur.wait_event(ev)
            _record_streams(lay, cur)
            _record_streams(g, cur)
            for t in g._prefetched_bonds:
                t.record_stream(cur)
            return lay, g
    return None


class StackContext:

    def __init__(self, model, X, Hin, batch_id, segment_id, mask, is_global, compound_edge_index, LAS_edge_index, coord_LAS):
        if not X.is_cuda:
            raise RuntimeError("fabind_amd: the docking stack runs on a HIP device only (no CPU fallback); got "
                               + str(X.device))
        args = model.args
        self.model = model
        self.scale = float(args.coordinate_scale)
        self.step = float(args.geometry_reg_step_size)
        self.clampv = 10.0 / self.scale
        self.P = prepare_stack_params(model)
        pre = _take_prefetched(X, batch_id) if _PREFETCHED else None
# ... 90 lines not shown
```

### fabind_amd/kernels.py

```python
import ctypes

import numpy as np
import torch

from . import _lib
from . import config as _cfg
from ._lib import ACT_NONE, ACT_RELU, ACT_SIGMOID, ACT_SILU, ACT_STORED_DERIV, GemmArgs, check, dt_code, ptr, stream

__all__ = ["gemm", "colsum", "edges_count", "edges_fill", "exclusive_scan", "inter_meta",
           "edge_geom", "gcl_pre", "segment_sum", "coord_update", "cross_attn_fwd", "pair_bmat", "pair_hadamard",
           "inter_attn_fwd", "las_step", "select_rows", "ACT_NONE", "ACT_SILU", "ACT_RELU", "ACT_SIGMOID", "ACT_STORED_DERIV"]

GEMM_BN = 128
GEMM_DEFAULT_CONFIG = 13
PROFILE = None
PROFILE_ONLY = None


PROFILE_BYTES = {}
PROFILE_ALGO = {}


def _profiled(label, flops, fn, nbytes=0.0, algo=None):
    if PROFILE is None or (PROFILE_ONLY is not None and not label.startswith(PROFILE_ONLY)):
        return fn()
    e0, e1 = torch.cuda.Event(enable_timing=True), torch.cuda.Event(enable_timing=True)
    e0.record()
    r = fn()
    e1.record()
    PROFILE.setdefault(label, []).append((e0, e1, flops))
    PROFILE_BYTES[label] = PROFILE_BYTES.get(label, 0.0) + float(nbytes)
    PROFILE_ALGO[label] = PROFILE_ALGO.get(label, 0.0) + float(nbytes if algo is None else algo)
    return r


def _split3():
    from .config import get_precision
    return get_precision() == "bf16x3"


def _ld(t):
    assert t.stride(-1) == 1 or t.shape[-1] == 1, "innermost dimension must be contiguous"
    return t.stride(0) if t.dim() == 2 else t.shape[-1]


def gemm(A, W, bias=None, A2=None, act_pro=ACT_NONE, act_epi=ACT_NONE, residual=None, r_index=None,
         out=None, out_dtype=torch.float32, want_out=True, dotvec=None, aux=None, dact=ACT_NONE, alpha=1.0,
         accumulate=False, groups=None, n_groups=0, max_m=0, max_n=0, M=None, N=None, ldc=None, k_splits=1,
         out2=None, groups_ext=False, p_drop=0.0, seed=0, out16=None, flops=None, force_x3=False):
    lib = _lib.load()
    a = GemmArgs()
    K1 = A.shape[1]
    K = K1 + (A2.shape[1] if A2 is not None else 0)
    M = A.shape[0] if M is None else M
    N = W.shape[0] if N is None else N
    assert groups_ext or W.shape[1] == K, "gemm: K mismatch %s vs %s" % (tuple(W.shape), K)
    if want_out and out is None:
        out = torch.empty((k_splits, M, N) if k_splits > 1 else (M, N), dtype=out_dtype, device=A.device)
        if k_splits > 1:
            ldc = N
    dot_out = None
    if dotvec is not None:
        nt = (N + GEMM_BN - 1) // GEMM_BN
        dot_out = torch.empty((A.shape[0], nt), dtype=torch.float32, device=A.device)
        a.dot_ld = nt
    a.A, a.A2, a.W, a.C = ptr(A), ptr(A2), ptr(W), ptr(out) if want_out else None
    a.bias, a.R, a.r_index = ptr(bias), ptr(residual), ptr(r_index)
    a.dotvec, a.dot_out, a.aux, a.groups = ptr(dotvec), ptr(dot_out), ptr(aux), ptr(groups)
    a.C2 = ptr(out2)
    a.c2_bf16 = 1 if (out2 is not None and want_out and out2.dtype == torch.bfloat16 and out.dtype == torch.float32) else 0
    if out16 is not None:
        a.C16, a.ldc16 = ptr(out16), _ld(out16)
    a.M, a.N, a.K, a.K1 = M, N, K, K1
    a.lda, a.lda2, a.ldw = _ld(A), (_ld(A2) if A2 is not None else 0), _ld(W)
    a.ldc = (ldc if ldc is not None else (_ld(out) if want_out else 0))
    a.ldr = _ld(residual) if residual is not None else 0
    a.r_dtype = dt_code(residual.dtype) if residual is not None else 0
    a.ldaux = _ld(aux) if aux is not None else 0
    a.a_dtype, a.w_dtype = dt_code(A.dtype), dt_code(W.dtype)
    a.c_dtype = dt_code(out.dtype) if want_out else 0
    a.aux_dtype = dt_code(aux.dtype) if aux is not None else 0
    if A2 is not None:
        assert A2.dtype == A.dtype
    a.act_pro, a.act_epi, a.dact_epi = act_pro, act_epi, dact
    a.accumulate = 1 if accumulate else 0
    a.n_groups, a.max_m, a.max_n = n_groups, max_m, max_n
    a.k_splits = k_splits
    a.groups_ext = 1 if groups_ext else 0
    a.alpha = alpha
    a.p_drop, a.drop_seed = float(p_drop), int(seed) & 0xFFFFFFFF
    x3 = A.dtype == torch.float32 and W.dtype == torch.float32 and (_split3() or force_x3)
    a.split3 = 1 if x3 else 0
    if PROFILE is None:
        check(lib.fabind_gemm(ctypes.byref(a), stream()), "fabind_gemm")
        return (out if want_out else None), dot_out
    label = "%s <%s,%s%s> M=%d N=%d K=%d" % ("fabind_gemm_x3" if x3 else "fabind_gemm", str(A.dtype).replace("torch.", ""),
                                             str(W.dtype).replace("torch.", ""), ",x3" if x3 else "", M, N, K)
    if groups is not None:
        label += " (ragged, %d groups)" % n_groups
    nb = 0.0
    if groups is None:
        mn = float(M) * N
        nb = float(M) * K * A.element_size() + float(N) * K * W.element_size()
        nb += mn * out.element_size() * (2 if accumulate else 1) if want_out else 0.0
        for t_ in (out2, residual, aux):
            if t_ is not None:
                nb += mn * t_.element_size()
        if out16 is not None:
            nb += mn * 2
    _profiled(label, 2.0 * M * N * K if flops is None else float(flops),
              lambda: check(lib.fabind_gemm(ctypes.byref(a), stream()), "fabind_gemm"), nb)
    return (out if want_out else None), dot_out


def colsum(x, out=None, accumulate=False):
    R, C = x.shape
    nchunk = max(1, min(1024, (R + 255) // 256))
    scratch = torch.empty((nchunk, C), dtype=torch.float32, device=x.device)
    if out is None:
        out = torch.empty((C,), dtype=torch.float32, device=x.device)
        accumulate = False
    check(_lib.load().fabind_colsum(ptr(x), dt_code(x.dtype), _ld(x), ptr(out), R, C, 1 if accumulate else 0,
                                    ptr(scratch), nchunk, stream()), "fabind_colsum")
    return out


def edges_count(x, node_off, c_cnt, B, max_n, bond_row, bond_off, cut_intra, cut_inter):
    N = x.shape[0]
    deg_ctx = torch.empty(N, dtype=torch.int32, device=x.device)
    deg_int = torch.empty(N, dtype=torch.int32, device=x.device)
    check(_lib.load().fabind_edges_count(ptr(x), ptr(node_off), ptr(c_cnt), B, max_n, ptr(bond_row), ptr(bond_off),
                                         cut_intra, cut_inter, ptr(deg_ctx), ptr(deg_int), stream()), "fabind_edges_count")
    return deg_ctx, deg_int


def exclusive_scan(deg):
    out = torch.empty(deg.shape[0] + 1, dtype=torch.int32, device=deg.device)
    check(_lib.load().fabind_exclusive_scan(ptr(deg), ptr(out), deg.shape[0], stream()), "fabind_exclusive_scan")
    return out


def edges_fill(x, node_off, c_cnt, B, max_n, bond_row, bond_col, bond_off, cut_intra, cut_inter, rowptr_ctx, rowptr_int,
               E_ctx, E_int):
    dev = x.device
    col_ctx = torch.empty(max(E_ctx, 1), dtype=torch.int32, device=dev)
    row_ctx = torch.empty(max(E_ctx, 1), dtype=torch.int32, device=dev)
    col_int = torch.empty(max(E_int, 1), dtype=torch.int32, device=dev)
    row_int = torch.empty(max(E_int, 1), dtype=torch.int32, device=dev)
    check(_lib.load().fabind_edges_fill(ptr(x), ptr(node_off), ptr(c_cnt), B, max_n, ptr(bond_row), ptr(bond_col),
                                        ptr(bond_off), cut_intra, cut_inter, ptr(rowptr_ctx), ptr(rowptr_int),
                                        ptr(col_ctx), ptr(row_ctx), ptr(col_int), ptr(row_int), stream()),
          "fabind_edges_fill")
    return col_ctx[:E_ctx], row_ctx[:E_ctx], col_int[:E_int], row_int[:E_int]


def inter_meta(node_off, c_cnt, B, rowptr_int, col_int, row_int):
    dev = col_int.device
    E = col_int.shape[0]
    red_off = torch.empty(B + 1, dtype=torch.int32, device=dev)
    red_idx = torch.empty(max(E, 1), dtype=torch.int32, device=dev)
    n_red = E // 2
    red_c = torch.empty(max(n_red, 1), dtype=torch.int32, device=dev)
    red_p = torch.empty(max(n_red, 1), dtype=torch.int32, device=dev)
    mirror = torch.empty(max(E, 1), dtype=torch.int32, device=dev)
    check(_lib.load().fabind_inter_meta(ptr(node_off), ptr(c_cnt), B, ptr(rowptr_int), ptr(col_int), ptr(row_int), E,
                                        ptr(red_off), ptr(red_idx), ptr(red_c), ptr(red_p), ptr(mirror), stream()),
          "fabind_inter_meta")
    return red_off, red_idx[:E], red_c[:n_red], red_p[:n_red], mirror[:E]


def edge_geom(x, row, col, rowptr, node_off, B):
    E, dev = row.shape[0], x.device
    d = torch.empty((max(E, 1), 3), dtype=torch.float32, device=dev)
    rho = torch.empty(max(E, 1), dtype=torch.float32, device=dev)
    rhohat = torch.empty(max(E, 1), dtype=torch.float32, device=dev)
# ... 819 lines not shown
```

### fabind_amd/ops.py

```python
import ctypes

import numpy as np
import torch

from . import config as _cfg
from . import kernels as K
from ._lib import GemmArgs, check, dt_code, load, ptr, stream


def act_dtype():
    return torch.float32 if _cfg.fp32_storage() else torch.bfloat16


mm_dtype = act_dtype


def needs_grad(*ts):
    return torch.is_grad_enabled() and any(torch.is_tensor(t) and t.requires_grad for t in ts)


_needs_grad = needs_grad


def _nchunk(rows):
# ... 75 lines not shown
    if path == "x3_tn":
        dW, db = _tn(dpre.to(torch.bfloat16), _b16(x), _b16(x2) if x2 is not None else None, W, with_db)
    elif path == "tn":
        dW, db = _tn(dpre, x, x2, W, with_db)
    else:
        S, Rp = _ksplit(dpre.shape[0])
        dpt, xt = _transposed(dpre, Rp), _transposed(x, Rp)
        if x2 is not None:
            xt = torch.cat([xt, _transposed(x2, Rp)], 0)
        if S == 1:
            dW = K.gemm(dpt, xt)[0]
        else:
            part, _ = K.gemm(dpt, xt, k_splits=S)
            dW = K.colsum(part.reshape(S, -1)).reshape(part.shape[1], part.shape[2])
        dW, db = dW.to(W.dtype), None
    if want_db and db is None:
        db = K.colsum(dpre)
    return dW, db


def _param_grads(dpre, x, x2, W, want_dW, want_db, db=None):
    dW = None
    if want_dW:
        dW, db_ = _weight_grad(dpre, x, x2, W, want_db and db is None)
        db = db if db is not None else db_
    elif want_db and db is None:
        db = K.colsum(dpre)
    return dW, (db if want_db else None)


def _mul_dact(dy, aux, act, out_dtype, scale=1.0):
    out = torch.empty(dy.shape, dtype=out_dtype, device=dy.device)
    a = aux if aux is not None else dy
    check(load().fabind_mul_dact(ptr(dy), dt_code(dy.dtype), ptr(a), dt_code(a.dtype), act, ptr(out), dt_code(out_dtype),
                                 dy.numel(), float(scale), stream()), "fabind_mul_dact")
    return out


DB_IN_TN_ROWS = 32768


def _db_in_tn(dy):
    return K.TN_DEFER and dy.shape[0] <= DB_IN_TN_ROWS and dy.dtype in (torch.float32, torch.bfloat16) and mm_dtype() == torch.bfloat16


def _mul_dact_colsum(dy, aux, act, out_dtype, scale=1.0):
    R, C = dy.shape
    out = torch.empty((R, C), dtype=out_dtype, device=dy.device)
    nchunk = max(1, min(4096, (R + 63) // 64))
    scratch = torch.empty((nchunk, C), dtype=torch.float32, device=dy.device)
    db = torch.empty(C, dtype=torch.float32, device=dy.device)
    check(load().fabind_mul_dact_colsum(ptr(dy), dt_code(dy.dtype), ptr(aux), dt_code(aux.dtype) if aux is not None else 0,
                                        act, ptr(out), dt_code(out_dtype), R, C, ptr(db), ptr(scratch), nchunk, float(scale), stream()),
          "fabind_mul_dact_colsum")
    return out, db


def _mul_dropmask_colsum(dy, p_drop, seed, out_dtype):
    R, C = dy.shape
    out = torch.empty((R, C), dtype=out_dtype, device=dy.device)
    nchunk = max(1, min(4096, (R + 63) // 64))
    scratch = torch.empty((nchunk, C), dtype=torch.float32, device=dy.device)
    db = torch.empty(C, dtype=torch.float32, device=dy.device)
    check(load().fabind_mul_dropmask_colsum(ptr(dy), dt_code(dy.dtype), ptr(out), dt_code(out_dtype), R, C, float(p_drop), int(seed) & 0xFFFFFFFF,
                                            ptr(db), ptr(scratch), nchunk, stream()), "fabind_mul_dropmask_colsum")
    return out, db


def _dpre_plan(dy, act, drop, want_db, want_dW):
    if drop is not None:
        return "dropmask", bool(want_db)
    kind = "act" if act != K.ACT_NONE else "cast" if dy.dtype != mm_dtype() else "none"
    return kind, bool(want_db and kind != "none" and dy.dim() == 2 and dy.shape[1] % 4 == 0 and not (want_dW and _db_in_tn(dy)))


def _dpre(dy, act, aux, scale, drop, want_db, want_dW):
    kind, with_db = _dpre_plan(dy, act, drop, want_db, want_dW)
    md = mm_dtype()
    if kind == "dropmask":
        dpre, db = _mul_dropmask_colsum(dy, drop[0], drop[1], md)
        return dpre, (db if with_db else None)
    if kind == "none":
        return dy, None
    scale = scale if kind == "act" else 1.0
    return _mul_dact_colsum(dy, aux, act, md, scale) if with_db else (_mul_dact(dy, aux, act, md, scale), None)


def _mm_in(x):
    return _b16(x) if (x is not None and _cfg.get_precision() == "bf16" and x.dtype == torch.float32) else x


def _stored_wt(W):
    t = getattr(W, "_fab_T", None)
    return t if (t is not None and t.shape == (W.shape[1], W.shape[0])) else None


def _wt(Wt, W):
    return Wt if Wt is not None else W.t().contiguous()


def _padded_k(dpre, W, Wt, Np):
    N = W.shape[0]
    if Np == N:
        return dpre, _wt(Wt, W)
    Wp = torch.zeros((W.shape[1], Np), dtype=W.dtype, device=W.device)
    Wp[:, :N] = W.t()
    dp = torch.zeros((dpre.shape[0], Np), dtype=dpre.dtype, device=dpre.device)
    dp[:, :N] = dpre
    return dp, Wp


def _drop_scale(p_drop):
    return 1.0 / (1.0 - int(p_drop * 65536.0 + 0.5) / 65536.0)


def _drop_seed(p_drop):
    return int(torch.randint(0, 2 ** 31 - 1, (1,)).item()) if p_drop > 0.0 else 0


def _attach_b16(y, y16):
    if y16 is not None:
        y._fab_b16 = (y._version, y16)
    return y


def _want16(out_dtype, act_epi, want):
    return bool(want) and _cfg.get_precision() in ("bf16", "bf16x3") and out_dtype == torch.float32 and act_epi == K.ACT_NONE


class _Linear(torch.autograd.Function):
    @staticmethod
    def forward(ctx, x, W, b, x2, residual, act_epi, out_dtype, holder=None, p_drop=0.0, seed=0, W32=None):
        assert act_epi in (K.ACT_NONE, K.ACT_RELU, K.ACT_SILU)
        drop_regen = p_drop > 0.0 and act_epi == K.ACT_NONE
        assert p_drop == 0.0 or (act_epi == K.ACT_RELU and residual is None) or \
            (drop_regen and out_dtype == torch.float32 and x2 is None and W32 is None and W.shape[0] % 4 == 0), \
            "epilogue dropout under autograd: ReLU without a residual, or no activation with an fp32 output"
        ctx.drop_scale = _drop_scale(p_drop)
        ctx.drop_regen = (float(p_drop), int(seed)) if drop_regen else None
        xin, x2in = _mm_in(x), _mm_in(x2)
        D = None
        M, N = x.shape[0], W.shape[0]
        y = torch.empty((M, N), dtype=out_dtype, device=x.device)
        relu_res = act_epi == K.ACT_RELU and residual is not None
        if act_epi == K.ACT_SILU or relu_res:
            D = torch.empty((M, N), dtype=out_dtype, device=x.device)
        y16 = None
        if holder is not None:
            y16 = torch.empty((M, N), dtype=torch.bfloat16, device=x.device)
            holder.append(y16)
        _linear_fwd(x, xin, x2, x2in, W, W32, b, y, act_epi=act_epi, residual=residual, D=D, y16=y16, p_drop=p_drop, seed=seed)
        ctx.act_epi, ctx.x_dtype = (K.ACT_SILU if relu_res else act_epi), x.dtype
        ctx.x2_dtype = x2.dtype if x2 is not None else None
        ctx.has_b, ctx.has_res, ctx.has_x2 = b is not None, residual is not None, x2 is not None
        ctx.res_dtype = residual.dtype if residual is not None else None
        ctx.sink_x, ctx.sink_res = _sink_of(x), _sink_of(residual)
        ctx.x_shape = x.shape
        ctx.save_for_backward(xin, W, x2in, y if (act_epi == K.ACT_RELU and not relu_res) else None, D)
        ctx.Wt = _stored_wt(W)
        return y

    @staticmethod
    def backward(ctx, dy):
        x, W, x2, y, D = ctx.saved_tensors
        dy = dy.contiguous()
        want_dW, want_db = ctx.needs_input_grad[1], ctx.has_b and ctx.needs_input_grad[2]
        act = K.ACT_STORED_DERIV if ctx.act_epi == K.ACT_SILU else ctx.act_epi
        aux = y if ctx.act_epi == K.ACT_RELU else D
        dpre, db = _dpre(dy, act, aux, ctx.drop_scale, ctx.drop_regen, want_db, want_dW)
        K1, N = x.shape[1], W.shape[0]
        dx = dx2 = None
        sink_x = ctx.sink_x if (ctx.x_dtype in (torch.float32, torch.bfloat16) and ctx.needs_input_grad[0]) else None
        if ctx.needs_input_grad[0] or (ctx.has_x2 and ctx.needs_input_grad[3]):
            pad64 = N % 64 != 0 and N <= 64 and dpre.shape[0] >= 65536 and dpre.dtype == torch.bfloat16
            dmm, Wt = _padded_k(dpre, W, ctx.Wt, 64 if pad64 else (N + 7) // 8 * 8)
            if sink_x is not None:
                dx = sink_x.gemm_into(dmm, Wt[:K1], x, ctx.x_dtype)
                if ctx.has_x2 and ctx.needs_input_grad[3]:
                    dx2, _ = K.gemm(dmm, Wt[K1:], out_dtype=torch.float32 if ctx.x2_dtype == torch.float32 else ctx.x2_dtype)
            else:
                dfull, _ = K.gemm(dmm, Wt, out_dtype=torch.float32 if ctx.x_dtype == torch.float32 else ctx.x_dtype)
                if ctx.has_x2:
                    dx, dx2 = dfull[:, :K1], dfull[:, K1:]
                    if ctx.x2_dtype != dx2.dtype:
                        dx2 = dx2.to(ctx.x2_dtype)
                else:
                    dx = dfull
        dW, db = _param_grads(dpre, x, x2, W, want_dW, want_db, db)
        dres = None
        if ctx.has_res and ctx.needs_input_grad[4]:
            dres = dy if dy.dtype == ctx.res_dtype else dy.to(ctx.res_dtype)
        if dres is not None and ctx.sink_res is not None:
            dres = ctx.sink_res.deposit(dres)
        return dx, dW, db, dx2, dres, None, None, None, None, None, None


def _gemm_split_rows(x, xin, W, W32, b, y, y16):
    W32p, lo, hi = W32
    N = W.shape[0]
    for a_, b_ in ((0, lo), (hi, N)):
        if b_ > a_:
            K.gemm(xin, W[a_:b_], bias=b[a_:b_] if b is not None else None, out=y[:, a_:b_], out16=y16[:, a_:b_] if y16 is not None else None)
    K.gemm(x, W32p, bias=b[lo:hi] if b is not None else None, out=y[:, lo:hi], out16=y16[:, lo:hi] if y16 is not None else None, force_x3=True)


def _linear_fwd(x, xin, x2, x2in, W, W32, b, y, act_pro=K.ACT_NONE, act_epi=K.ACT_NONE, residual=None, D=None, y16=None, p_drop=0.0, seed=0):
    if isinstance(W32, tuple):
        _gemm_split_rows(x, xin, W, W32, b, y, y16)
    elif W32 is not None:
        K.gemm(x, W32, bias=b, A2=x2, act_epi=act_epi, residual=residual, out=y, out2=D, out16=y16, p_drop=p_drop, seed=seed, force_x3=True)
    else:
        K.gemm(xin, W, bias=b, A2=x2in, act_pro=act_pro, act_epi=act_epi, residual=residual, out=y, out2=D, out16=y16, p_drop=p_drop, seed=seed)


def _split_site_ok(x, W, W32, x2, act_pro, out_dtype, p_drop, act_epi=K.ACT_NONE, residual=None):
    if W32 is None or _cfg.get_precision() != "bf16" or x.dtype != torch.float32 or act_pro != K.ACT_NONE or out_dtype != torch.float32 \
            or p_drop != 0.0 or x.stride(0) % 4 != 0 or x.data_ptr() % 16 != 0:
        return False
    if isinstance(W32, tuple):
        W32p, lo, hi = W32
        return (W32p.dtype == torch.float32 and W32p.stride(-1) == 1 and tuple(W32p.shape) == (hi - lo, W.shape[1]) and 0 <= lo < hi <= W.shape[0]
                and lo % 128 == 0 and hi % 128 == 0 and x2 is None and act_epi == K.ACT_NONE and residual is None)
    return (W32.dtype == torch.float32 and tuple(W32.shape) == tuple(W.shape) and W32.stride(-1) == 1 and (x2 is None or x2.dtype == torch.float32))


def linear(x, W, b=None, act_pro=K.ACT_NONE, act_epi=K.ACT_NONE, residual=None, x2=None, out_dtype=torch.float32,
           p_drop=0.0, want16=False, W32=None):
    if x.stride(-1) != 1:
        x = x.contiguous()
    seed = _drop_seed(p_drop)
    if not _split_site_ok(x, W, W32, x2, act_pro, out_dtype, p_drop, act_epi, residual):
        W32 = None
    if _needs_grad(x, W, b, x2, residual):
        assert act_pro == K.ACT_NONE, "producer-side activations only under autograd"
        K.tn_hook(W, b)
        holder = [] if _want16(out_dtype, act_epi, want16) else None
        y = _Linear.apply(x, W, b, x2, residual, act_epi, out_dtype, holder, p_drop, seed, W32)
        return _attach_b16(y, holder[0] if holder else None)
    y16 = None
    if _want16(out_dtype, act_epi, want16) and act_pro == K.ACT_NONE and (p_drop == 0.0 or (act_epi == K.ACT_NONE and x2 is None and W.shape[0] % 4 == 0)):
        y16 = torch.empty((x.shape[0], W.shape[0]), dtype=torch.bfloat16, device=x.device)
    y = torch.empty((x.shape[0], W.shape[0]), dtype=out_dtype, device=x.device)
    xin, x2in = (_mm_in(x), _mm_in(x2)) if (W32 is None or isinstance(W32, tuple)) else (None, None)
    _linear_fwd(x, xin, x2, x2in, W, W32, b, y, act_pro, act_epi, residual, y16=y16, p_drop=p_drop, seed=seed)
    return _attach_b16(y, y16)


class _MLP2(torch.autograd.Function):

    @staticmethod
    def forward(ctx, x, x2, W1, b1, W2, b2, residual, act, holder=None, p_drop=0.0, seed=0, W32=None, chain=None):
        assert act in (K.ACT_RELU, K.ACT_SILU)
        ctx.drop = (float(p_drop), int(seed)) if p_drop > 0.0 else None
        xin, x2in = _mm_in(x), _mm_in(x2)
        M, N1 = x.shape[0], W1.shape[0]
        ad = act_dtype()
        split_ok = W32 is not None and ctx.drop is None and _split_site_ok(x, W1, W32[0], x2, K.ACT_NONE, torch.float32, 0.0, act, None)
        if split_ok and chain is not None and _chain_ok(x, x2, residual, W1, W2):
            y, y16, t, D = K.node_chain_x3_fwd(x, x2, chain, b1.float(), b2.float(), act, 0 if x2 is not None else 1, residual=residual,
                                               want16=holder is not None, save=True)
        else:
            y16 = torch.empty((M, W2.shape[0]), dtype=torch.bfloat16, device=x.device) if holder is not None else None
            t = torch.empty((M, N1), dtype=ad, device=x.device)
            D = torch.empty((M, N1), dtype=ad, device=x.device) if act == K.ACT_SILU else None
            if split_ok:
                t32 = torch.empty((M, N1), dtype=torch.float32, device=x.device)
                K.gemm(x, W32[0], bias=b1, A2=x2, act_epi=act, out=t32, out2=D, out16=t, force_x3=True)
                y, _ = K.gemm(t32, W32[1], bias=b2, residual=residual, out_dtype=torch.float32, out16=y16, force_x3=True)
                del t32
            else:
                K.gemm(xin, W1, bias=b1, A2=x2in, act_epi=act, out=t, out2=D)
                y, _ = K.gemm(t, W2, bias=b2, residual=residual, out_dtype=torch.float32, out16=y16, p_drop=p_drop, seed=seed)
        if holder is not None:
            holder.append(y16)
        ctx.act, ctx.has_x2, ctx.has_res = act, x2 is not None, residual is not None
        ctx.res_is_x = residual is x
        ctx.sink_x, ctx.sink_res = _sink_of(x), _sink_of(residual)
        ctx.x2_dtype = x2.dtype if x2 is not None else None
        ctx.save_for_backward(xin, x2in, W1, W2, t, D)
        ctx.W1t, ctx.W2t = _stored_wt(W1), _stored_wt(W2)
        return y

    @staticmethod
    def backward(ctx, dy):
        xin, x2in, W1, W2, t, D = ctx.saved_tensors
        dy = dy.contiguous()
        ni = ctx.needs_input_grad
        dy16, db2 = _dpre(dy, K.ACT_NONE, None, 1.0, ctx.drop, ni[5], ni[4])
        dW2, db2 = _param_grads(dy16, t, None, W2, ni[4], ni[5], db2)
        aux, dact = (t, K.ACT_RELU) if ctx.act == K.ACT_RELU else (D, K.ACT_STORED_DERIV)
        dmm, W2t = _padded_k(dy16, W2, ctx.W2t, (W2.shape[0] + 7) // 8 * 8)
        dpre, _ = K.gemm(dmm, W2t, aux=aux, dact=dact, out_dtype=mm_dtype())
        dW1, db1 = _param_grads(dpre, xin, x2in, W1, ni[2], ni[3])
        W1t = _wt(ctx.W1t, W1)
        K1 = xin.shape[1]
        dres = dy if (ctx.has_res and ni[6]) else None
        dx = dx2 = None
        if ni[0]:
            if ctx.sink_x is not None:
                if dres is not None and ctx.sink_res is ctx.sink_x:
                    ctx.sink_x.deposit(dres)
                    dres = None
                dx = ctx.sink_x.gemm_into(dpre, W1t[:K1], xin)
            elif dres is not None and ctx.res_is_x:
                dx, _ = K.gemm(dpre, W1t[:K1], residual=dres, out_dtype=torch.float32)
                dres = None
            else:
                dx, _ = K.gemm(dpre, W1t[:K1], out_dtype=torch.float32)
        if dres is not None and ctx.sink_res is not None:
            dres = ctx.sink_res.deposit(dres)
        if ctx.has_x2 and ni[1]:
            dx2, _ = K.gemm(dpre, W1t[K1:], out_dtype=torch.float32 if ctx.x2_dtype == torch.float32 else ctx.x2_dtype)
        return dx, dx2, dW1, db1, dW2, db2, dres, None, None, None, None, None, None


def _chain_ok(x, x2, residual, W1, W2):
    H = W2.shape[0]
    ok = lambda t: t.dtype == torch.float32 and t.dim() == 2 and t.shape[1] == H and t.stride(1) == 1 and t.stride(0) % 4 == 0 and t.data_ptr() % 16 == 0
    kind0 = x2 is not None
    return (H in (128, 256, 512) and ok(x) and (x2 is None or ok(x2)) and (residual is None or ok(residual))
            and tuple(W1.shape) == ((H, 2 * H) if kind0 else (2 * H, H)) and tuple(W2.shape) == ((H, H) if kind0 else (H, 2 * H)))


def mlp2(x, W1, b1, act, W2, b2, residual=None, x2=None, want16=False, p_drop=0.0, W32=None, chain=None):
    if W32 is not None and (W32[0] is None or W32[1] is None or p_drop != 0.0 or _cfg.get_precision() != "bf16"):
        W32 = None
    if _needs_grad(x, x2, W1, b1, W2, b2, residual):
        K.tn_hook(W1, b1, W2, b2)
        holder = [] if _want16(torch.float32, K.ACT_NONE, want16) else None
        y = _MLP2.apply(x, x2, W1, b1, W2, b2, residual, act, holder, p_drop, _drop_seed(p_drop), W32, chain if W32 is not None else None)
        return _attach_b16(y, holder[0] if holder else None)
    if W32 is not None:
        t = linear(x, W1, b1, act_epi=act, x2=x2, out_dtype=torch.float32, W32=W32[0])
        return linear(t, W2, b2, residual=residual, want16=want16, W32=W32[1])
    t = linear(x, W1, b1, act_epi=act, x2=x2, out_dtype=act_dtype())
    return linear(t, W2, b2, residual=residual, want16=want16, p_drop=p_drop)


class _MLP2Relu(torch.autograd.Function):

    @staticmethod
    def forward(ctx, x, W1, b1, W2, b2, residual, last_act, out_dtype, p_drop, seed1, seed2):
        assert not (last_act and residual is not None), "relu + dropout on the output: the residual is added by the caller"
        ctx.drop_scale = _drop_scale(p_drop)
        ad = act_dtype()
        M = x.shape[0]
        t = torch.empty((M, W1.shape[0]), dtype=ad, device=x.device)
        K.gemm(x, W1, bias=b1, act_epi=K.ACT_RELU, out=t, p_drop=p_drop, seed=seed1)
        y = torch.empty((M, W2.shape[0]), dtype=out_dtype, device=x.device)
        if last_act:
            K.gemm(t, W2, bias=b2, act_epi=K.ACT_RELU, out=y, p_drop=p_drop, seed=seed2)
        else:
            K.gemm(t, W2, bias=b2, residual=residual, out=y)
        ctx.last_act, ctx.has_res = last_act, residual is not None
        ctx.res_dtype = residual.dtype if residual is not None else None
        ctx.sink_res = _sink_of(residual)
        ctx.save_for_backward(x, W1, W2, t, y if last_act else None)
        ctx.W1t, ctx.W2t = _stored_wt(W1), _stored_wt(W2)
        return y

    @staticmethod
    def backward(ctx, dy):
        x, W1, W2, t, y = ctx.saved_tensors
        dy = dy.contiguous()
        ni = ctx.needs_input_grad
        s = ctx.drop_scale
        dpre2, db2 = _dpre(dy, K.ACT_RELU if ctx.last_act else K.ACT_NONE, y, s, None, ni[4], ni[3])
        dW2, db2 = _param_grads(dpre2, t, None, W2, ni[3], ni[4], db2)
        dpre1, _ = K.gemm(dpre2, _wt(ctx.W2t, W2), aux=t, dact=K.ACT_RELU, alpha=s, out_dtype=mm_dtype())
        dW1, db1 = _param_grads(dpre1, x, None, W1, ni[1], ni[2])
        dx = K.gemm(dpre1, _wt(ctx.W1t, W1), out_dtype=x.dtype)[0] if ni[0] else None
        dres = None
        if ctx.has_res and ni[5]:
            dres = dy if dy.dtype == ctx.res_dtype else dy.to(ctx.res_dtype)
            if ctx.sink_res is not None:
                dres = ctx.sink_res.deposit(dres)
        return dx, dW1, db1, dW2, db2, dres, None, None, None, None, None


def mlp2_relu(x, W1, b1, W2, b2, last_act, residual=None, out_dtype=torch.float32, p_drop=0.0):
    seeds = torch.randint(0, 2 ** 31 - 1, (2,)).tolist() if p_drop > 0.0 else (0, 0)
    K.tn_hook(W1, b1, W2, b2)
    return _MLP2Relu.apply(x, W1, b1, W2, b2, residual, last_act, out_dtype, p_drop, int(seeds[0]), int(seeds[1]))


def _gemm_rowdot(x, W, b, u, act_pro, act_epi, store, p_drop=0.0, seed=0, fold=None, post=False):
    M, Kd = x.shape
    N = W.shape[0]
    nt = (N + K.GEMM_BN - 1) // K.GEMM_BN
    part = torch.empty((M, nt), dtype=torch.float32, device=x.device)
    z = torch.empty((M, N), dtype=act_dtype(), device=x.device) if store else None
    a = GemmArgs()
    a.A, a.W, a.C, a.bias, a.dotvec, a.dot_out = ptr(x), ptr(W), ptr(z), ptr(b), ptr(u), ptr(part)
    a.M, a.N, a.K, a.K1 = M, N, Kd, Kd
    a.lda, a.ldw, a.ldc, a.dot_ld = x.stride(0), W.stride(0), N, nt
    a.a_dtype, a.w_dtype, a.c_dtype = dt_code(x.dtype), dt_code(W.dtype), dt_code(z.dtype) if store else 0
    a.act_pro, a.act_epi, a.store_preact, a.alpha = act_pro, act_epi, (0 if post else 1), 1.0
    a.p_drop, a.drop_seed = float(p_drop), int(seed) & 0xFFFFFFFF
    if fold is not None:
        a.store_preact = 0
        a.row_mu, a.row_rs, a.col_c = ptr(fold[0]), ptr(fold[1]), ptr(fold[2])
    x3 = x.dtype == torch.float32 and W.dtype == torch.float32 and _cfg.get_precision() == "bf16x3"
    a.split3 = 1 if x3 else 0
    label = "%s <%s,%s%s> M=%d N=%d K=%d" % ("fabind_gemm_x3" if x3 else "fabind_gemm", str(x.dtype).replace("torch.", ""),
                                             str(W.dtype).replace("torch.", ""), ",x3" if x3 else "", M, N, Kd)
    K._profiled(label, 2.0 * M * N * Kd, lambda: check(load().fabind_gemm(ctypes.byref(a), stream()), "fabind_gemm(rowdot)"))
    return z, part


def _rowdot_bwd(z, dpart, u, act_epi):
    M, N = z.shape
    dz = torch.empty_like(z)
    nchunk = _nchunk(M)
    scratch = torch.empty((nchunk, N), dtype=torch.float32, device=z.device)
# ... 342 lines not shown

    @staticmethod
    def backward(ctx, d_rows):
        idx, = ctx.saved_tensors
        n, w = ctx.n, ctx.w
        srt, perm = torch.sort(idx, stable=True)
        ptr = torch.searchsorted(srt, torch.arange(n + 1, dtype=idx.dtype, device=idx.device)).to(torch.int32)
        g8 = torch.zeros((d_rows.shape[0], 8), dtype=torch.float32, device=d_rows.device)
        g8[:, :w] = d_rows
        out = K.segment_sum(g8, ptr, n, eidx=perm.to(torch.int32))
        return out[:, :w].to(d_rows.dtype), None


def take_rows_few(x, index64):
    if _needs_grad(x) and x.dim() == 2 and x.shape[1] <= 8 and x.dtype == torch.float32 and index64.numel() > 0:
        return _TakeRowsFew.apply(x, index64)
    return x.index_select(0, index64)


class _DropMix(torch.autograd.Function):

    @staticmethod
    def forward(ctx, h, hn, p_drop, seed):
        out = torch.empty_like(h)
        check(load().fabind_drop_mix(ptr(h), ptr(hn), ptr(out), h.numel(), float(p_drop), int(seed) & 0xFFFFFFFF, stream()), "fabind_drop_mix")
        ctx.pd, ctx.seed = float(p_drop), int(seed)
        return out

    @staticmethod
    def backward(ctx, g):
        g = g.contiguous()
        dhn, dh = torch.empty_like(g), torch.empty_like(g)
        check(load().fabind_drop_mix_bwd(ptr(g), ptr(dhn), ptr(dh), g.numel(), ctx.pd, ctx.seed & 0xFFFFFFFF, stream()), "fabind_drop_mix_bwd")
        return dh, dhn, None, None


def drop_mix(h, hn, p_drop):
    if p_drop <= 0.0:
        return hn
    if (h.dtype == torch.float32 and hn.dtype == torch.float32 and h.is_contiguous() and hn.is_contiguous() and h.shape == hn.shape
            and h.numel() % 4 == 0 and h.is_cuda):
        seed = _drop_seed(p_drop)
        if _needs_grad(h, hn):
            return _DropMix.apply(h, hn, p_drop, seed)
        out = torch.empty_like(h)
        check(load().fabind_drop_mix(ptr(h), ptr(hn), ptr(out), h.numel(), float(p_drop), seed, stream()), "fabind_drop_mix")
        return out
    return h + torch.nn.functional.dropout(hn - h, p_drop, True)


def sum_sorted_segments(x, counts):
    return torch.segment_reduce(x.detach(), "sum", lengths=counts.to(torch.int64), axis=0)


def take_unique_rows(x, index64):
    return _TakeUniqueRows.apply(x, index64) if _needs_grad(x) else x.index_select(0, index64)


def take_rows(x, index64):
    sink = _sink_of(x)
    if sink is not None and _needs_grad(x):
        return _TakeRows.apply(x, index64, sink)
    return x.index_select(0, index64)


class _PutRows(torch.autograd.Function):

    @staticmethod
    def forward(ctx, base, rows, idx, inplace):
        ctx.save_for_backward(idx)
        if not inplace:
            out = base.clone()
            out.index_copy_(0, idx, rows.to(base.dtype))
            return out
        _put_rows_inplace(base, rows, idx)
        ctx.mark_dirty(base)
        return base

    @staticmethod
    def backward(ctx, dout):
        idx, = ctx.saved_tensors
        d_rows = dout.index_select(0, idx)
        if dout.is_contiguous() and _owned_grad(dout):
            d_base = dout
            d_base.index_fill_(0, idx, 0.0)
        else:
            d_base = dout.index_fill(0, idx, 0.0)
        return d_base, d_rows, None, None


def _owned_grad(g):
    return bool(getattr(g, "_fab_owned", False)) and g._use_count() <= 2


def _put_rows_inplace(base, rows, idx):
    c = getattr(base, "_fab_b16", None)
    keep = c is not None and c[0] == base._version
    base.index_copy_(0, idx, rows.to(base.dtype))
    if keep:
        c[1].index_copy_(0, idx, rows.to(torch.bfloat16))
        base._fab_b16 = (base._version, c[1])


def put_rows(base, rows, index64, inplace=True):
    if _needs_grad(base, rows):
        c = getattr(base, "_fab_b16", None)
        keep = c is not None and c[0] == base._version
        out = _PutRows.apply(base, rows, index64, inplace)
        if keep and inplace:
            out._fab_b16 = (out._version, c[1])
        return out
    _put_rows_inplace(base, rows, index64)
    return base


def select_rows(x, z, mask_u8):
    if _needs_grad(x, z):
        return torch.where(mask_u8.bool()[:, None], z, x)
    return K.select_rows(x, z, mask_u8)


class GradSink:

    def __init__(self):
        self.buf = None
        self.pending = None
        self.rows = []
        self.deferred = []

    def take(self, like):
        if self.buf is None:
            self.buf = torch.zeros_like(like)
            self._flush_into_buf()
            return self.buf, True
        return self.buf, False

    def _flush_into_buf(self):
        if self.pending is not None:
            self.buf.add_(self.pending)
            self.pending = None
        for idx, r in self.rows:
            self.buf.index_add_(0, idx, r.to(self.buf.dtype))
        self.rows = []

    def deposit(self, g):
        if self.buf is not None:
            self.buf.add_(g)
        elif self.pending is None:
            self.pending = g
        else:
            self.pending = self.pending + g
        return None

    def deposit_rows(self, idx, rows):
        if self.buf is not None:
            self.buf.index_add_(0, idx, rows.to(self.buf.dtype))
        else:
            self.rows.append((idx, rows))
        return None

    def gemm_into(self, A, Wt, like, dtype=torch.float32):
        if (A.dtype == torch.bfloat16 and Wt.dtype == torch.bfloat16 and A.dim() == 2 and A.stride(1) == 1 and A.stride(0) % 8 == 0
                and A.shape[1] % 64 == 0 and A.shape[0] >= DEFER_DX_MIN_ROWS and A.data_ptr() % 16 == 0):
            self.deferred.append((A, Wt))
            return None
        if self.buf is None:
            out = torch.empty(like.shape, dtype=dtype, device=like.device)
            pend = self.pending
            if pend is not None and pend.dtype != out.dtype and not (pend.dtype == torch.bfloat16 and out.dtype == torch.float32):
                pend = pend.to(out.dtype)
            K.gemm(A, Wt, out=out, residual=pend)
            self.pending = None
            self.buf = out
            rows, self.rows = self.rows, []
            for idx, r in rows:
                out.index_add_(0, idx, r.to(out.dtype))
            return out
        K.gemm(A, Wt, out=self.buf, accumulate=True)
        return None


DEFER_DX_MIN_ROWS = 1024


def _run_deferred(defs, out, base, accumulate):
    defs = sorted(defs, key=lambda d_: -d_[0].shape[1])
    first = True
    while defs:
        if len(defs) >= 2:
            (A1, W1), (A2, W2) = defs[0], defs[1]
            defs = defs[2:]
            Wcat = torch.cat([W1, W2], 1)
            args = dict(A2=A2)
        else:
            (A1, Wcat), = defs
            defs, args = [], {}
        if first and not accumulate:
            K.gemm(A1, Wcat, out=out, residual=base, **args)
        else:
            K.gemm(A1, Wcat, out=out, accumulate=True, **args)
        first = False


class _SinkOwner(torch.autograd.Function):
    @staticmethod
    def forward(ctx, t, sink):
        ctx.sink = sink
        ctx.meta = (t.shape, t.dtype, t.device)
        ctx.set_materialize_grads(False)
        return t.view_as(t)

    @staticmethod
    def backward(ctx, g):
        sink = ctx.sink
        pend, rows, defs = sink.pending, sink.rows, sink.deferred
        owned = g is not None and g is sink.buf
        sink.buf, sink.pending, sink.rows, sink.deferred = None, None, [], []
        if defs:
            if owned:
                _run_deferred(defs, g, None, True)
            else:
                base = g
                if pend is not None:
                    base, pend = (pend if base is None else base + pend), None
                if base is not None and base.dtype != ctx.meta[1] and not (base.dtype == torch.bfloat16 and ctx.meta[1] == torch.float32):
                    base = base.to(ctx.meta[1])
                g = torch.empty(ctx.meta[0], dtype=ctx.meta[1], device=ctx.meta[2])
                _run_deferred(defs, g, base, False)
                owned = True
        if pend is not None:
            if g is None:
                g, owned = pend, False
            else:
                g, owned = g + pend, True
        if rows:
            if g is None:
                g = torch.zeros(ctx.meta[0], dtype=ctx.meta[1], device=ctx.meta[2])
            elif not owned:
                g = g.clone()
            owned = True
            for idx, r in rows:
                g.index_add_(0, idx, r.to(g.dtype))
        if owned:
            g._fab_owned = True
        return g, None


def shared_grad(t):
    if not (torch.is_grad_enabled() and t.requires_grad):
        return t
    sink = GradSink()
    out = _SinkOwner.apply(t, sink)
    out._fab_gsink = sink
    c = getattr(t, "_fab_b16", None)
    if c is not None and c[0] == t._version:
        out._fab_b16 = (out._version, c[1])
    return out


def _sink_of(t):
    return getattr(t, "_fab_gsink", None) if t is not None else None


def _sink_zeros(t, sink):
    if sink is None:
        buf = torch.zeros_like(t)
        return buf, buf
    buf, first = sink.take(t)
    return buf, (buf if first else None)


class _CrossAttn(torch.autograd.Function):
    @staticmethod
    def forward(ctx, qg, kv, bias, lin_col, gate_col, desc, B, max_nq, max_nk, scale):
        out = torch.zeros((qg.shape[0], 128), dtype=torch.float32, device=qg.device)
        _, lse = K.cross_attn_fwd(qg[:, :128], kv[:, :128], kv[:, 128:], qg[:, 128:], bias, lin_col, gate_col, desc, B,
                                  max_nq, scale, out, want_lse=True, max_nk=max_nk)
        ctx.args = (lin_col, gate_col, desc, B, max_nq, max_nk, scale)
        ctx.mfma = K.cross_attn_use_mfma()
        ctx.covers_all = bool(getattr(desc, "_fab_covers_all", False))
        ctx.save_for_backward(qg, kv, bias, out, lse)
        return out

    @staticmethod
    def backward(ctx, dout):
        qg, kv, bias, out, lse = ctx.saved_tensors
        lin_col, gate_col, desc, B, max_nq, max_nk, scale = ctx.args
        dout = dout.contiguous()
        dqg, dkv = torch.zeros_like(qg), torch.zeros_like(kv)
        dbias = torch.empty_like(bias) if (bias.shape[1] == 8 and lin_col == 0 and gate_col == 4 and ctx.covers_all) else torch.zeros_like(bias)
        dO = torch.empty((qg.shape[0], 128), dtype=torch.float32, device=qg.device)
        Dv = torch.empty((qg.shape[0], 4), dtype=torch.float32, device=qg.device)
        n_scr = int(load().fabind_cross_attn_bwd_scratch(B, max_nq, max_nk))
        scr = torch.empty(n_scr, dtype=torch.float32, device=qg.device) if n_scr else None
        fn = load().fabind_cross_attn_mfma_bwd if ctx.mfma else load().fabind_cross_attn_bwd
        check(fn(ptr(qg), qg.stride(0), ptr(kv), kv.stride(0), ptr(bias), bias.stride(0), lin_col, gate_col, ptr(desc), B, max_nq,
                 max_nk, scale, ptr(out), ptr(lse), ptr(dout), ptr(dqg), ptr(dkv), ptr(dbias), ptr(dO), ptr(Dv), ptr(scr), stream()),
              "fabind_cross_attn_bwd")
        return dqg, dkv, dbias, None, None, None, None, None, None, None


def cross_attn(qg, kv, bias, lin_col, gate_col, desc, B, max_nq, max_nk, scale):
    if _needs_grad(qg, kv, bias):
        return _CrossAttn.apply(qg, kv, bias, lin_col, gate_col, desc, B, max_nq, max_nk, scale)
    out = torch.zeros((qg.shape[0], 128), dtype=torch.float32, device=qg.device)
    K.cross_attn_fwd(qg[:, :128], kv[:, :128], kv[:, 128:], qg[:, 128:], bias, lin_col, gate_col, desc, B, max_nq, scale, out,
                     max_nk=max_nk)
    return out


class _PairHadamard(torch.autograd.Function):

    @staticmethod
    def forward(ctx, T0, T1, H, H2, red_p, red_c, graph):
        ctx.dims = (H, H2)
        ctx.sink = getattr(T0, "_fab_gsink", None)
        ctx.graph = graph
        ctx.save_for_backward(T0, T1, red_p, red_c)
        return K.pair_hadamard(T0[:, :H], T0[:, H:], T1[:, :H2], T1[:, H2:], red_p, red_c, act_dtype())

    @staticmethod
    def backward(ctx, dhd):
        T0, T1, red_p, red_c = ctx.saved_tensors
        H, H2 = ctx.dims
        dhd = dhd.contiguous()
        d0, d0_ret = _sink_zeros(T0, ctx.sink)
        d1 = torch.zeros_like(T1)
        g = ctx.graph
        if (PAIRHAD_ROWS and g is not None and T0.dtype == torch.float32 and T1.dtype == torch.float32 and H % 4 == 0 and H2 % 4 == 0
                and H <= 1024 and H2 <= 256
                and dhd.stride(0) % 4 == 0):
            check(load().fabind_pair_hadamard_bwd_rows(
                ptr(dhd), dt_code(dhd.dtype), dhd.stride(0), ptr(T0), T0.stride(0), H, ptr(T1), T1.stride(0), H2, ptr(g.rp_int),
                ptr(g.col_int), ptr(g.red_idx), ptr(red_c), T0.shape[0], ptr(d0), d0.stride(0), ptr(d1), d1.stride(0), stream()),
# ... 28 lines not shown
        return K.pair_hadamard(t, t, dummy, dummy, ia, ib, act_dtype())

    @staticmethod
    def backward(ctx, dout):
        t, ia, ib = ctx.saved_tensors
        dout = dout.contiguous()
        W = t.shape[1]
        bl = ctx.blocks
        if bl is not None and dout.dtype == torch.bfloat16 and t.dtype == torch.float32 and W in (64, 128, 256, 512) and t.stride(0) % 2 == 0 \
                and ctx.n_a == bl.n_prows and t.shape[0] == bl.n_prows + bl.n_crows and dout.shape[0] == bl.n_pairs:
            dt_ = torch.empty_like(t)
            part = torch.empty((bl.n_tiles, bl.nchunk_max, bl.chunk, W), dtype=torch.float32, device=t.device)
            tc, dtc = t[ctx.n_a:], dt_[ctx.n_a:]
            check(load().fabind_block_hadamard_bwd(bl.desc_ptr, bl.B, bl.n_tiles, ptr(dout), dout.stride(0), ptr(t), t.stride(0), ptr(tc),
                                                   t.stride(0), W, bl.row_b_ptr, bl.n_crows, bl.nchunk_max, ptr(part), ptr(dt_),
                                                   dt_.stride(0), ptr(dtc), dt_.stride(0), stream()), "fabind_block_hadamard_bwd")
            return dt_, None, None, None, None, None
        if ROWS_HADAMARD_WALK and t.dtype == torch.float32 and W % 4 == 0 and W <= 1024 and t.stride(0) % 4 == 0 and dout.stride(0) % 4 == 0:
            n = t.shape[0]
            rowptr, pair_idx, partner = _rows_hadamard_csr(ia, ib, n, ctx.a_sorted)
            dt_ = torch.empty_like(t)
            check(load().fabind_rows_hadamard_bwd(ptr(dout), dt_code(dout.dtype), dout.stride(0), ptr(t), t.stride(0), W,
                                                  ptr(rowptr), ptr(pair_idx), ptr(partner), n, ptr(dt_), dt_.stride(0),
                                                  stream()), "fabind_rows_hadamard_bwd")
            return dt_, None, None, None, None, None
        dt_ = torch.zeros_like(t)
        check(load().fabind_pair_hadamard_bwd(ptr(dout), dt_code(dout.dtype), dout.stride(0), ptr(t), ptr(t), t.stride(0), W,
                                              None, None, 0, 0, ptr(ia), ptr(ib), ia.shape[0], ptr(dt_), ptr(dt_),
                                              dt_.stride(0), None, None, 0, stream()), "fabind_pair_hadamard_bwd")
        return dt_, None, None, None, None, None


def _rows_hadamard_csr(ia, ib, n, a_sorted=False):
    P = ia.shape[0]
    dev = ia.device
    ia64, ib64 = ia.long(), ib.long()
    pa = torch.arange(P, device=dev) if a_sorted else torch.argsort(ia64, stable=True)
    pb = torch.argsort(ib64, stable=True)
    one = torch.ones_like(ia64)
    ca = torch.zeros(n, dtype=torch.int64, device=dev).index_add_(0, ia64, one)
    cb_ = torch.zeros(n, dtype=torch.int64, device=dev).index_add_(0, ib64, one)
    rowptr = torch.zeros(n + 1, dtype=torch.int64, device=dev)
    rowptr[1:] = torch.cumsum(ca + cb_, 0)
    starts = rowptr[:-1]
    sa, sb = ia64[pa], ib64[pb]
    ar = torch.arange(P, device=dev)
    ra = ar - (torch.cumsum(ca, 0) - ca)[sa]
    rb = ar - (torch.cumsum(cb_, 0) - cb_)[sb]
    pair_idx = torch.empty(2 * P, dtype=torch.int32, device=dev)
    partner = torch.empty(2 * P, dtype=torch.int32, device=dev)
    posa, posb = starts[sa] + ra, starts[sb] + ca[sb] + rb
    pair_idx[posa], partner[posa] = pa.to(torch.int32), ib64[pa].to(torch.int32)
    pair_idx[posb], partner[posb] = pb.to(torch.int32), ia64[pb].to(torch.int32)
    return rowptr.to(torch.int32), pair_idx, partner


ROWS_HADAMARD_WALK = _cfg.knob("FABIND_ROWS_HADAMARD_WALK")


def _block_hadamard_fwd(t, bl, n_a):
    W = t.shape[1]
    if not (bl is not None and act_dtype() == torch.bfloat16 and t.dtype == torch.float32 and W in (64, 128, 256, 512) and t.stride(1) == 1
            and t.stride(0) % 4 == 0 and t.data_ptr() % 16 == 0 and n_a == bl.n_prows and t.shape[0] == bl.n_prows + bl.n_crows and n_a % 4 == 0):
        return None
    out = torch.empty((bl.n_pairs, W), dtype=torch.bfloat16, device=t.device)
    check(load().fabind_block_hadamard_fwd(bl.desc_ptr, bl.B, bl.n_tiles, ptr(t), t.stride(0), ptr(t[n_a:]), t.stride(0), W, ptr(out), W,
                                           stream()), "fabind_block_hadamard_fwd")
    return out


def rows_hadamard(t, idx_a, idx_b, a_sorted=False, blocks=None, n_a=0):
    ia, ib = idx_a.to(torch.int32).contiguous(), idx_b.to(torch.int32).contiguous()
    if _needs_grad(t):
        return _RowsHadamard.apply(t, ia, ib, a_sorted, blocks, n_a)
    fwd = _block_hadamard_fwd(t, blocks, n_a)
    if fwd is not None:
        return fwd
    dummy = t[:, :0]
    return K.pair_hadamard(t, t, dummy, dummy, ia, ib, act_dtype())


class _InterAttn(torch.autograd.Function):
    @staticmethod
    def forward(ctx, qkv, cv, h, x, d, rhohat, bias_part, w_rk, w_rv, wcr, w3, H, g, clampv, s_ext=None, Wc=None, bc=None, holder=None, Wc32=None):
        v_in = None
        if Wc is not None:
            c16 = getattr(qkv, "_fab_b16", None) if _cfg.get_precision() == "bf16" else None
            v_in = c16[1][:, 2 * H:] if (c16 is not None and c16[0] == qkv._version) else _mm_in(qkv[:, 2 * H:])
            if Wc32 is not None:
                cv, _ = K.gemm(qkv[:, 2 * H:], Wc32, bias=bc, force_x3=True)
            else:
                cv, _ = K.gemm(v_in, Wc, bias=bc)
        h16 = None
        if holder is not None:
            h16 = torch.empty((h.shape[0], H), dtype=torch.bfloat16, device=h.device)
            holder.append(h16)
        h_out, x_out, alpha, cvs = K.inter_attn_fwd(qkv, cv, H, h, x, d, rhohat, g.rp_int, g.col_int, g.red_idx,
                                                    bias_part, w_rk, w_rv, wcr, w3, clampv, s_ext, h16, deal=getattr(g, "int_deal", None))
        ctx.g, ctx.H, ctx.clampv, ctx.np = g, H, clampv, bias_part.shape[1]
        ctx.has_ext, ctx.has_cv = s_ext is not None, Wc is not None
        ctx.sink_h, ctx.Wct = _sink_of(h), (_stored_wt(Wc) if Wc is not None else None)
        ctx.save_for_backward(qkv, cv, d, rhohat, w_rk, w_rv, wcr, w3, alpha, cvs, v_in, Wc)
        ctx.mark_non_differentiable(alpha)
        return h_out, x_out, alpha

    @staticmethod
    def backward(ctx, dh_out, dx_out, _dalpha):
        qkv, cv, d, rhohat, w_rk, w_rv, wcr, w3, alpha, cvs, v_in, Wc = ctx.saved_tensors
        g, H = ctx.g, ctx.H
        N, E = qkv.shape[0], g.col_int.shape[0]
        dev = qkv.device
        f32 = dict(dtype=torch.float32, device=dev)
        dh_out = dh_out.contiguous() if dh_out is not None else torch.zeros((N, H), **f32)
        dx_out = dx_out.contiguous() if dx_out is not None else torch.zeros((N, 3), **f32)
        dqkv = torch.empty_like(qkv)
        dcv = torch.empty_like(cv)
        dd, drh = torch.empty((max(E, 1), 3), **f32), torch.empty(max(E, 1), **f32)
        n_red = E // 2
        dbias_red = torch.zeros(max(n_red, 1), **f32)
        dlogit, dcp = torch.empty(max(E, 1), **f32), torch.empty(max(E, 1), **f32)
        if E == 0:
            dd.zero_(); drh.zero_()
        nblk = min((N + 3) // 4, INTER_BWD_BLOCKS)
        wpart = torch.empty((nblk, 4 * H), **f32)
        deal = getattr(g, "int_deal", None) if K.INTER_ATTN_ROWS else None
        if deal is not None:
            check(load().fabind_inter_attn_bwd_rows(ptr(qkv), qkv.stride(0), ptr(cv), cv.stride(0), H, ptr(d), ptr(rhohat),
                                                    ptr(g.rp_int), ptr(g.col_int), ptr(g.mirror), ptr(g.red_idx), ptr(w_rk),
                                                    ptr(w_rv), ptr(wcr), ptr(w3), ptr(alpha), ptr(cvs), ctx.clampv, N, ptr(dh_out),
                                                    ptr(dx_out), ptr(dqkv), ptr(dcv), ptr(dd), ptr(drh), ptr(dbias_red), ptr(dlogit),
                                                    ptr(dcp), ptr(wpart), nblk, ptr(deal[0]), int(deal[1]), int(deal[2]), stream()),
                  "fabind_inter_attn_bwd_rows")
        else:
            check(load().fabind_inter_attn_bwd(ptr(qkv), qkv.stride(0), ptr(cv), cv.stride(0), H, ptr(d), ptr(rhohat),
                                               ptr(g.rp_int), ptr(g.col_int), ptr(g.mirror), ptr(g.red_idx), ptr(w_rk),
                                               ptr(w_rv), ptr(wcr), ptr(w3), ptr(alpha), ptr(cvs), ctx.clampv, N, ptr(dh_out),
                                               ptr(dx_out), ptr(dqkv), ptr(dcv), ptr(dd), ptr(drh), ptr(dbias_red), ptr(dlogit),
                                               ptr(dcp), ptr(wpart), nblk, stream()), "fabind_inter_attn_bwd")
        dw_all = K.colsum(wpart)
        dw = [dw_all[i * H:(i + 1) * H] for i in range(4)]
        dWc = dbc = None
        if ctx.has_cv:
            ni = ctx.needs_input_grad
            dpre, dbc = _dpre(dcv, K.ACT_NONE, None, 1.0, None, ni[16], ni[15])
            K.gemm(dpre, _wt(ctx.Wct, Wc), out=dqkv[:, 2 * H:], accumulate=True)
            dWc, dbc = _param_grads(dpre, v_in, None, Wc, ni[15], ni[16], dbc)
            dcv = None
        if ctx.sink_h is not None and ctx.needs_input_grad[2]:
            dh_out = ctx.sink_h.deposit(dh_out)
        return (dqkv, dcv, dh_out, dx_out, dd[:E], drh[:E], dbias_red[:n_red, None].expand(n_red, ctx.np), dw[0], dw[1],
                dw[2], dw[3], None, None, None, dcp[:E] if ctx.has_ext else None, dWc, dbc, None, None)


INTER_BWD_BLOCKS = 1024


def inter_attn(qkv, cv, H, h, x, d, rhohat, g, bias_part, w_rk, w_rv, wcr, w3, clampv, s_ext=None, Wc=None, bc=None, own_h=False, Wc32=None):
    assert (cv is None) != (Wc is None), "inter_attn: pass either cv or its Linear (Wc, bc)"
    w16 = _cfg.get_precision() == "bf16" and h.is_contiguous()
    if Wc32 is not None and not (Wc is not None and _cfg.get_precision() == "bf16" and qkv.dtype == torch.float32 and Wc32.dtype == torch.float32
                                 and tuple(Wc32.shape) == tuple(Wc.shape) and qkv.stride(0) % 4 == 0):
        Wc32 = None
    if _needs_grad(qkv, cv, h, x, d, rhohat, bias_part, w_rk, w_rv, wcr, w3, s_ext, Wc, bc):
        K.tn_hook(Wc, bc)
        holder = [] if w16 else None
        h_out, x_out, alpha = _InterAttn.apply(qkv, cv, h, x, d, rhohat, bias_part, w_rk, w_rv, wcr, w3, H, g, clampv, s_ext, Wc, bc, holder, Wc32)
        return _attach_b16(h_out, holder[0] if holder else None), x_out, alpha
    if cv is None:
        cv = linear(qkv[:, 2 * H:], Wc, bc, W32=Wc32)
    deal = getattr(g, "int_deal", None)
    if own_h and deal is not None and K.INTER_ATTN_ROWS and h.is_contiguous() and h.dtype == torch.float32 and not h.requires_grad:
        c = getattr(h, "_fab_b16", None)
        h16 = (c[1] if (c is not None and c[0] == h._version and c[1].is_contiguous()) else h.to(torch.bfloat16)) if w16 else None
        h_out, x_out, alpha, _ = K.inter_attn_fwd(qkv, cv, H, h, x, d, rhohat, g.rp_int, g.col_int, g.red_idx, bias_part,
                                                  w_rk, w_rv, wcr, w3, clampv, s_ext, h16, deal=deal, inplace=True)
        return _attach_b16(h_out, h16), x_out, alpha
    h16 = torch.empty((h.shape[0], H), dtype=torch.bfloat16, device=h.device) if w16 else None
    h_out, x_out, alpha, _ = K.inter_attn_fwd(qkv, cv, H, h, x, d, rhohat, g.rp_int, g.col_int, g.red_idx, bias_part,
                                              w_rk, w_rv, wcr, w3, clampv, s_ext, h16, deal=deal)
    return _attach_b16(h_out, h16), x_out, alpha


class _LasStep(torch.autograd.Function):
    @staticmethod
    def forward(ctx, x, x0, las, lay, step, clampv):
        out, mask = K.las_step(x, x0, las[0], las[1], las[2], lay.node_off, lay.c_cnt, lay.B, lay.max_n, step, clampv, want_mask=True)
        ctx.las, ctx.lay, ctx.step, ctx.clampv = las, lay, step, clampv
        ctx.save_for_backward(x, x0, mask)
        return out

    @staticmethod
    def backward(ctx, dout):
        x, x0, mask = ctx.saved_tensors
        las, lay = ctx.las, ctx.lay
        dout = dout.contiguous()
        dx = torch.empty_like(x)
        check(load().fabind_las_step_bwd(ptr(x), ptr(x0), ptr(mask), ptr(las[0]), ptr(las[1]), ptr(las[2]),
                                         ptr(lay.node_off), ptr(lay.c_cnt), lay.B, lay.max_n, ctx.step, ctx.clampv,
                                         ptr(dout), ptr(dx), stream()), "fabind_las_step_bwd")
        return dx, None, None, None, None, None


def las_step(x, x0, las, lay, step, clampv):
    if _needs_grad(x):
        return _LasStep.apply(x, x0, las, lay, step, clampv)
    return K.las_step(x, x0, las[0], las[1], las[2], lay.node_off, lay.c_cnt, lay.B, lay.max_n, step, clampv)


def _pair_bias_fwd(a0b0, H, wcomp, bconst, lay):
    nblk, NO, _ = wcomp.shape
    outs = []
    a0 = a0b0[:, :H].to(torch.bfloat16) if mm_dtype() == torch.bfloat16 else a0b0[:, :H]
    for k in range(nblk):
        bmat = K.pair_bmat(a0b0[:, H:], wcomp[k], lay.c_index, mm_dtype())
        out = torch.empty((lay.n_pairs, NO), dtype=torch.float32, device=a0b0.device)
        K.gemm(a0, bmat, bias=bconst[k].repeat(lay.sumC), out=out, groups=lay.pb_groups, n_groups=lay.B,
               max_m=lay.max_P, max_n=lay.pb_max_n, M=lay.N, N=bmat.shape[0], ldc=NO, flops=2.0 * lay.n_pairs * NO * H)
        outs.append(out)
    return outs


def _pair_bias_groups(lay, H, ld_ab, nblk, Kp):
    key = ("pbg", H, ld_ab, nblk, Kp)
    if getattr(lay, "_pbg_key", None) != key:
        import numpy as np
        from .param_pack import upload
        B, NO = lay.B, 8
        dev = lay.node_off.device
        P, C = np.asarray(lay.P, dtype=np.int64), np.asarray(lay.C, dtype=np.int64)
        off, coff = np.asarray(lay.off[:-1], dtype=np.int64), np.asarray(lay.coff[:-1], dtype=np.int64)
        poff = np.concatenate([[0], np.cumsum(P)])[:-1]
        bb = np.arange(B, dtype=np.int64)
        lo = lambda v: (v & 0xFFFFFFFF)
        hi = lambda v: v >> 32
        zero = np.zeros(B, dtype=np.int64)
        co = (off + C) * ld_ab
        cat = np.stack([poff, P, bb * H, np.full(B, H), lo(co), hi(co), np.full(B, ld_ab), zero], 1)
        ch = coff * NO * H
        tg = np.stack([bb * Kp, C * NO, bb * H, np.full(B, H), lo(ch), hi(ch), np.full(B, H), zero], 1)
        both = (np.concatenate([cat, tg], 0) & 0xFFFFFFFF).astype(np.uint32).view(np.int32)
        devt = upload(both, dev, torch.int32)
        lay._pbg = (devt[:B], devt[B:])
        lay._pbg_key = key
    return lay._pbg


class _PairBias(torch.autograd.Function):
    @staticmethod
    def forward(ctx, a0b0, wcomp, bconst, H, lay):
# ... 471 lines not shown
```

### include/fabind_hip.h

```cpp
#ifndef FABIND_HIP_H
#define FABIND_HIP_H

#include <stdint.h>

#ifdef __cplusplus
extern "C" {
#endif

#ifndef __HIP_PLATFORM_AMD__
typedef struct ihipStream_t* hipStream_t;
#endif

const char* fabind_last_error(void);
#define FABIND_ABI_VERSION 19
int fabind_abi_version(void);
int fabind_sizeof_args(int which);

typedef struct FabindGemmArgs {
    const void* A;
    const void* A2;
    const void* W;
    void* C;
    const float* bias;
    const void* R;
// ... 345 lines not shown
#define FB_ELF_WAVE1 0
#define FB_ELF_WAVE1_TAIL 1
#define FB_ELF_WAVE2_TAIL 2
#define FB_ELF_CHUNK 3
#define FB_ELF_COUNT 4
int fabind_edge_lnfold_form(int Kp, int H, int* edges_per_trip);
int fabind_edge_lnfold_blocks(int E);
#define FB_ELB_NPL1 0
#define FB_ELB_NPL2 1
#define FB_ELB_NPL3 2
#define FB_ELB_COUNT 3
int fabind_edge_lnfold_bwd_form(int Kp, int* edges_per_trip);
int fabind_inter_coord_fold_blocks(int E);

int fabind_add(const float* a, const float* b, float* out, long n, hipStream_t stream);

int fabind_mul_dact(const void* dy, int dy_dt, const void* y, int y_dt, int act, void* out, int out_dt, long n, float scale,
                    hipStream_t stream);
int fabind_mul_dact_colsum(const void* dy, int dy_dt, const void* y, int y_dt, int act, void* out, int out_dt, int R, int C,
                           float* colsum, float* scratch, int nchunk, float scale, hipStream_t stream);
int fabind_mul_dropmask_colsum(const void* dy, int dy_dt, void* out, int out_dt, int R, int C, float p_drop, unsigned seed,
                               float* colsum, float* scratch, int nchunk, hipStream_t stream);
int fabind_drop_mix(const float* h, const float* hn, float* out, long n, float p_drop, unsigned seed, hipStream_t stream);
int fabind_drop_mix_bwd(const float* g, float* dhn, float* dh, long n, float p_drop, unsigned seed, hipStream_t stream);
int fabind_rowdot_bwd(const void* z, int z_dt, const float* dpart, int np, const float* u, int act, int M, int N,
                      void* dz, float* du, float* scratch, int nchunk, hipStream_t stream);
int fabind_edge_geom_bwd(const float* d, const float* rho, const float* norm, const float* dd, const float* drhohat,
                         const int* row, const int* rowptr, const int* colptr ,
                         const int* perm , const int* node_off, int B, int E, int n_nodes, float* dx,
                         float* g_scratch , float* T_scratch , hipStream_t stream);
int fabind_gcl_pre_bwd(const void* dpre, int dt, int H, const float* rhohat, const float* w_r, int E, float* drh,
                       float* dw, float* scratch, int nchunk, hipStream_t stream);
int fabind_gather_dact(const float* dout, int ldo, const int* row, const void* Z, int z_dt, int act, void* dZ, int dz_dt,
                       int E, int H, hipStream_t stream);
int fabind_coord_update_bwd(const float* d, const float* s, const int* rowptr, int n_rows, int mean, float clampv,
                            const float* dxo, float* dd, float* ds, hipStream_t stream);
long fabind_cross_attn_bwd_scratch(int B, int max_nq, int max_nk);
int fabind_cross_attn_bwd(const float* qg, int ldq, const float* kv, int ldkv, const float* bias, int bias_ld,
                          int lin_col, int gate_col, const int* desc, int B, int max_nq, int max_nk, float scale,
                          const float* out, const float* lse, const float* dout, float* dqg, float* dkv, float* dbias,
                          float* dO, float* Dv, float* scratch, hipStream_t stream);
int fabind_cross_attn_mfma_bwd(const float* qg, int ldq, const float* kv, int ldkv, const float* bias, int bias_ld,
                               int lin_col, int gate_col, const int* desc, int B, int max_nq, int max_nk, float scale,
                               const float* out, const float* lse, const float* dout, float* dqg, float* dkv, float* dbias,
                               float* dO, float* Dv, float* scratch, hipStream_t stream);
long fabind_pair_bias_cat_parts(int B, int max_P);
int fabind_pair_bias_cat(const void* const* douts, int nblk, const int* desc_p, int B, int max_P, int Kp, void* Acat, int lda,
                         const float* b0, int ld_ab, const int* c_index, const float* wcomp, int H, void* BTcat, int ldb,
                         float* colpart, hipStream_t stream);
int fabind_pair_bias_btcat(const float* b0, int ld_ab, const int* c_index, const int* desc_p, const float* wcomp, int nblk, int H, int Kp,
                           void* BTcat, int ldb, int B, hipStream_t stream);
int fabind_batched_transpose_pad(const void* in, int ld_in, const int* desc, int B, int nsub, int cols, int Pp, void* out,
                                 hipStream_t stream);
int fabind_pair_hadamard_bwd(const void* dhd, int dt, int ldh, const float* a0, const float* b0, int ld0, int H,
                             const float* a1, const float* b1, int ld1, int H2, const int* red_p, const int* red_c, int n,
                             float* da0, float* db0, int ldd0, float* da1, float* db1, int ldd1, hipStream_t stream);
int fabind_pair_hadamard_bwd_grid(const void* dhd, int dt, int ldh, const float* T, int ldt, int W, const int* node_off,
                                  const int* c_cnt, const int* node_b, const int* desc_p, int n_nodes, float* dT, int lddt,
                                  hipStream_t stream);
int fabind_node_chain_fwd(const void* X1, int ld1, const void* X2, int ld2, const void* W1a, const void* W1b, const float* b1,
                          const void* W2a, const void* W2b, const float* b2, int act, int kind, const float* R, int ldr, float* out,
                          int ldo, void* out16, int ldo16, int M, int H, hipStream_t stream);
int fabind_node_chain_x3_fwd(const float* X1, int ld1, const float* X2, int ld2, const void* W1ah, const void* W1al, const void* W1bh,
                             const void* W1bl, const float* b1, const void* W2ah, const void* W2al, const void* W2bh, const void* W2bl,
                             const float* b2, int act, int kind, const float* R, int ldr, float* out, int ldo, void* out16, int ldo16,
                             void* t16, int ldt, void* d16, int ldd, int M, int H, hipStream_t stream);
int fabind_rows_hadamard_bwd(const void* dout, int dt, int ldo, const float* t, int ldt, int W, const int* rowptr, const int* pair_idx,
                             const int* partner, int n_rows, float* dT, int lddt, hipStream_t stream);
int fabind_pair_hadamard_bwd_rows(const void* dhd, int dt, int ldh, const float* t0, int ld0, int H, const float* t1, int ld1, int H2,
                                  const int* rowptr, const int* col, const int* red_idx, const int* red_c, int n_rows, float* d0,
                                  int ldd0, float* d1, int ldd1, hipStream_t stream);
int fabind_inter_attn_bwd(const float* qkv, int ldqkv, const float* cv, int ldcv, int H, const float* d,
                          const float* rhohat, const int* rowptr, const int* col, const int* mirror, const int* red_idx,
                          const float* w_rk, const float* w_rv, const float* wcr, const float* w3, const float* alpha,
                          const float* cvs, float clampv, int n_rows, const float* dh_out, const float* dx_out,
                          float* dqkv, float* dcv, float* dd, float* drh, float* dbias_red, float* dlogit, float* dcp,
                          float* wpart, int nblk, hipStream_t stream);
int fabind_inter_attn_bwd_rows(const float* qkv, int ldqkv, const float* cv, int ldcv, int H, const float* d,
                               const float* rhohat, const int* rowptr, const int* col, const int* mirror, const int* red_idx,
                               const float* w_rk, const float* w_rv, const float* wcr, const float* w3, const float* alpha,
                               const float* cvs, float clampv, int n_rows, const float* dh_out, const float* dx_out,
                               float* dqkv, float* dcv, float* dd, float* drh, float* dbias_red, float* dlogit, float* dcp,
                               float* wpart, int nblk, const int* order, int n_heavy, int n_act, hipStream_t stream);
int fabind_las_step_bwd(const float* x, const float* x0, const unsigned char* pass_mask, const int* las_i, const int* las_j,
                        const int* las_off, const int* node_off, const int* c_cnt, int B, int max_n, float step,
                        float clampv, const float* dout, float* dx, hipStream_t stream);
int fabind_pair_bias_bwd(const float* dout, int NO, const float* ab, int ld, int H, const float* w, const int* desc_p,
                         int B, int max_P, int max_C, const int* p_index, const int* c_index, float* dab, float* dwk,
                         hipStream_t stream);
int fabind_pair_bias_finish_parts(int n_c);
int fabind_pair_bias_finish(const float* T, const float* ab, int ld, int H, const float* w, const int* c_index, int n_c,
                            float* dab, float* dw_part, long ld_part, hipStream_t stream);
void fabind_gemm_set_config(int cfg);
void fabind_gemm_set_persistent(int on);
int fabind_gemm_x3_occupancy(int wm);
void fabind_cross_attn_fused_set_dbg(void* five_int64_on_device);
int fabind_cross_attn_fused_occupancy(int lds_bytes);
void fabind_gemm_set_x3_tile(int wm);
void fabind_gemm_set_small_m(int tiles);
void fabind_gemm_tn_set_waves(int waves);
int fabind_gemm_tn_tile_n(void);
void fabind_gemm_tn_set_exp(int mask);

#ifdef __cplusplus
}
#endif
#endif
```

Measured before the change: 536.9.

## Fuse qkv linear backward into inter-attn op with bf16 grads; merge segment-sum kernels

The inter-attention autograd op now optionally owns the qkv linear, so its backward writes dq/dk and dcv gradients directly in bf16. These feed the qkv and Wc weight-gradient GEMMs without fp32 round trips or separate autograd nodes. The dv part stays fp32 so the Wc GEMM can accumulate into it, and that GEMM also emits a bf16 copy. Separately, the light and heavy segment-sum kernels are merged into one 1024-thread launch that dispatches on block index, trading two launches for one at the cost of a larger block size for the light rows.

```diff
diff --git a/fabind_amd/_lib.py b/fabind_amd/_lib.py
--- a/fabind_amd/_lib.py
+++ b/fabind_amd/_lib.py
@@ -164,6 +164,8 @@
                               _vp, _vp, _vp, _vp, _vp, _vp, _vp, _vp, _vp, _vp, _i, _vp],
     "fabind_inter_attn_bwd_rows": [_vp, _i, _vp, _i, _i, _vp, _vp, _vp, _vp, _vp, _vp, _vp, _vp, _vp, _vp, _vp, _vp, _f, _i,
                                    _vp, _vp, _vp, _vp, _vp, _vp, _vp, _vp, _vp, _vp, _i, _vp, _i, _i, _vp],
+    "fabind_inter_attn_bwd_rows_b16": [_vp, _i, _vp, _i, _i, _vp, _vp, _vp, _vp, _vp, _vp, _vp, _vp, _vp, _vp, _vp, _vp, _f, _i,
+                                       _vp, _vp, _vp, _i, _vp, _i, _vp, _i, _vp, _vp, _vp, _vp, _vp, _vp, _i, _vp, _i, _i, _vp],
     "fabind_las_step_bwd": [_vp, _vp, _vp, _vp, _vp, _vp, _vp, _vp, _i, _i, _f, _f, _vp, _vp, _vp],
     "fabind_pair_bias_bwd": [_vp, _i, _vp, _i, _i, _vp, _vp, _i, _i, _i, _vp, _vp, _vp, _vp, _vp],
     "fabind_pair_bias_btcat": [_vp, _i, _vp, _vp, _vp, _i, _i, _i, _vp, _i, _i, _vp],
diff --git a/fabind_amd/csrc/gcl.hip b/fabind_amd/csrc/gcl.hip
--- a/fabind_amd/csrc/gcl.hip
+++ b/fabind_amd/csrc/gcl.hip
@@ -185,11 +185,11 @@
 }
 
 template <int NSLAB>
-__global__ __launch_bounds__(256) void segment_sum_kernel(const void* __restrict__ Z, int z_dt, int ldz, int H,
-                                                          const int* rowptr, const int* eidx, int act, float* out,
-                                                          int ldo, int n_rows, bf16_t* out16, int ldo16, int heavy_min) {
+__device__ __forceinline__ void segment_sum_light_rows(const void* __restrict__ Z, int z_dt, int ldz, int H, const int* rowptr,
+                                                       const int* eidx, int act, float* out, int ldo, int n_rows, bf16_t* out16,
+                                                       int ldo16, int heavy_min, int blk) {
     const int lane = threadIdx.x & 63;
-    const int r = blockIdx.x * 4 + (threadIdx.x >> 6);
+    const int r = blk * 16 + (threadIdx.x >> 6);
     if (r >= n_rows) return;
     const int e0 = rowptr[r], e1 = rowptr[r + 1];
     if (e1 - e0 > heavy_min) return;
@@ -214,16 +214,16 @@
 }
 
 template <int NSLAB>
-__global__ __launch_bounds__(1024) void segment_sum_heavy_kernel(const void* __restrict__ Z, int z_dt, int ldz, int H,
-                                                                 const int* rowptr, const int* eidx, int act, float* out,
-                                                                 int ldo, int n_rows, bf16_t* out16, int ldo16, int rpw, int heavy_min) {
+__device__ __forceinline__ void segment_sum_heavy_rows(const void* __restrict__ Z, int z_dt, int ldz, int H, const int* rowptr,
+                                                       const int* eidx, int act, float* out, int ldo, int n_rows, bf16_t* out16,
+                                                       int ldo16, int rpw, int heavy_min, int blk) {
     __shared__ F8 part[15][NSLAB * 64];
     __shared__ int heavy[1024];
     __shared__ int n_heavy;
     const int lane = threadIdx.x & 63, w = threadIdx.x >> 6;
     if (threadIdx.x == 0) n_heavy = 0;
     __syncthreads();
-    const int rr = blockIdx.x * rpw + threadIdx.x;
+    const int rr = blk * rpw + threadIdx.x;
     if ((int)threadIdx.x < rpw && rr < n_rows && rowptr[rr + 1] - rowptr[rr] > heavy_min) heavy[atomicAdd(&n_heavy, 1)] = rr;
     __syncthreads();
     const int nh = n_heavy;
@@ -261,6 +261,18 @@
         }
         __syncthreads();
     }
+}
+
+template <int NSLAB>
+__global__ __launch_bounds__(1024) void segment_sum_kernel(const void* __restrict__ Z, int z_dt, int ldz, int H,
+                                                           const int* rowptr, const int* eidx, int act, float* out,
+                                                           int ldo, int n_rows, bf16_t* out16, int ldo16, int rpw, int heavy_min,
+                                                           int n_heavy_wg) {
+    const int blk = (int)blockIdx.x;
+    if (blk < n_heavy_wg)
+        segment_sum_heavy_rows<NSLAB>(Z, z_dt, ldz, H, rowptr, eidx, act, out, ldo, n_rows, out16, ldo16, rpw, heavy_min, blk);
+    else
+        segment_sum_light_rows<NSLAB>(Z, z_dt, ldz, H, rowptr, eidx, act, out, ldo, n_rows, out16, ldo16, heavy_min, blk - n_heavy_wg);
 }
 
 extern "C" int fabind_segment_sum(const void* Z, int z_dt, int ldz, int H, const int* rowptr, const int* eidx,
@@ -277,14 +289,12 @@
     int rpw = 1024;
     while (rpw > 64 && (n_rows + rpw - 1) / rpw < 256) rpw >>= 1;
     const int heavy_min = n_rows < 16384 ? 32 : 128;
-    const dim3 g((n_rows + 3) / 4), gh((n_rows + rpw - 1) / rpw);
-    if (H <= 512) {
-        hipLaunchKernelGGL((segment_sum_kernel<1>), g, dim3(256), 0, stream, Z, z_dt, ldz, H, rowptr, eidx, act, out, ldo, n_rows, out16, ldo16, heavy_min);
-        hipLaunchKernelGGL((segment_sum_heavy_kernel<1>), gh, dim3(1024), 0, stream, Z, z_dt, ldz, H, rowptr, eidx, act, out, ldo, n_rows, out16, ldo16, rpw, heavy_min);
-    } else {
-        hipLaunchKernelGGL((segment_sum_kernel<2>), g, dim3(256), 0, stream, Z, z_dt, ldz, H, rowptr, eidx, act, out, ldo, n_rows, out16, ldo16, heavy_min);
-        hipLaunchKernelGGL((segment_sum_heavy_kernel<2>), gh, dim3(1024), 0, stream, Z, z_dt, ldz, H, rowptr, eidx, act, out, ldo, n_rows, out16, ldo16, rpw, heavy_min);
-    }
+    const int gh = (n_rows + rpw - 1) / rpw, gl = (n_rows + 15) / 16;
+    const dim3 g(gh + gl);
+    if (H <= 512)
+        hipLaunchKernelGGL((segment_sum_kernel<1>), g, dim3(1024), 0, stream, Z, z_dt, ldz, H, rowptr, eidx, act, out, ldo, n_rows, out16, ldo16, rpw, heavy_min, gh);
+    else
+        hipLaunchKernelGGL((segment_sum_kernel<2>), g, dim3(1024), 0, stream, Z, z_dt, ldz, H, rowptr, eidx, act, out, ldo, n_rows, out16, ldo16, rpw, heavy_min, gh);
     FB_CHECK_LAUNCH();
     return 0;
 }
diff --git a/fabind_amd/csrc/inter_attn_rows.hip b/fabind_amd/csrc/inter_attn_rows.hip
--- a/fabind_amd/csrc/inter_attn_rows.hip
+++ b/fabind_amd/csrc/inter_attn_rows.hip
@@ -204,13 +204,19 @@
     return 0;
 }
 
-template <int NS>
+template <bool O16>
+__device__ __forceinline__ void st_grad4(void* base, size_t off, const float4 v) {
+    if (O16) *(uint2*)((bf16_t*)base + off) = make_uint2(pack2_bf16(v.x, v.y), pack2_bf16(v.z, v.w));
+    else *(float4*)((float*)base + off) = v;
+}
+
+template <int NS, bool O16>
 __global__ __launch_bounds__(256) void inter_attn_bwd_a_rows_kernel(
     const float* __restrict__ qkv, int ldqkv, const float* __restrict__ cv, int ldcv, int H, const float* __restrict__ d,
     const float* __restrict__ rhohat, const int* rowptr, const int* col, const float* __restrict__ w_rk,
     const float* __restrict__ w_rv, const float* __restrict__ wcr, const float* __restrict__ w3, const float* alpha,
     const float* cvs, float clampv, int n_rows, const float* __restrict__ dh_out, const float* __restrict__ dx_out,
-    float* dqkv, float* dd, float* drh, float* dlogit, float* dcp, float* wpart, const int* __restrict__ order, int n_heavy, int n_act) {
+    void* dqkv, int ldo, float* dd, float* drh, float* dlogit, float* dcp, float* wpart, const int* __restrict__ order, int n_heavy, int n_act) {
     extern __shared__ float4 shp[];
     float (*sS)[4] = (float (*)[4])(shp + 4 * NS * 64);
     const int lane = threadIdx.x & 63, wv = threadIdx.x >> 6;
@@ -238,7 +244,7 @@
 #pragma unroll
             for (int s = 0; s < NS; ++s) {
                 const int c = s * 256 + lane * 4;
-                if (c < H) *(float4*)(dqkv + (size_t)r * ldqkv + c) = z4;
+                if (c < H) st_grad4<O16>(dqkv, (size_t)r * ldo + c, z4);
             }
             continue;
         }
@@ -379,7 +385,7 @@
             for (int s = 0; s < NS; ++s) {
                 const int c = s * 256 + lane * 4;
                 if (c < H) {
-                    *(float4*)(dqkv + (size_t)r * ldqkv + c) = dq[s];
+                    st_grad4<O16>(dqkv, (size_t)r * ldo + c, dq[s]);
                     a_wrk[s].x += s_lrh * qv[s].x; a_wrk[s].y += s_lrh * qv[s].y; a_wrk[s].z += s_lrh * qv[s].z; a_wrk[s].w += s_lrh * qv[s].w;
                     a_wrv[s].x += s_arh * gh[s].x; a_wrv[s].y += s_arh * gh[s].y; a_wrv[s].z += s_arh * gh[s].z; a_wrv[s].w += s_arh * gh[s].w;
                 }
@@ -398,7 +404,7 @@
                         const float4 o = shp[w * NS * 64 + g];
                         t.x += o.x; t.y += o.y; t.z += o.z; t.w += o.w;
                     }
-                    *(float4*)(dqkv + (size_t)r * ldqkv + c) = t;
+                    st_grad4<O16>(dqkv, (size_t)r * ldo + c, t);
                 }
             }
             if (wv == 0) {
@@ -435,12 +441,13 @@
     }
 }
 
-template <int NS>
+template <int NS, bool O16>
 __global__ __launch_bounds__(256) void inter_attn_bwd_b_rows_kernel(
     const float* __restrict__ qkv, int ldqkv, const float* __restrict__ cv, int ldcv, int H, const float* rhohat,
     const int* rowptr, const int* col, const int* mirror, const int* red_idx, const float* __restrict__ wcr,
     const float* __restrict__ w3, const float* alpha, const float* dlogit, const float* dcp, int n_rows,
-    const float* __restrict__ dh_out, float* dqkv, float* dcv, float* dbias_red, const int* __restrict__ order, int n_heavy, int n_act) {
+    const float* __restrict__ dh_out, void* dqkv, int ldo, float* dv, int lddv, void* dcv, int ldoc, float* dbias_red,
+    const int* __restrict__ order, int n_heavy, int n_act) {
     extern __shared__ float4 shb[];
     const int lane = threadIdx.x & 63, wv = threadIdx.x >> 6;
     const bool coop = (int)blockIdx.x < n_heavy;
@@ -448,11 +455,11 @@
     if (idx >= n_rows) return;
     const int n = order[idx];
     const float4 z4 = make_float4(0.f, 0.f, 0.f, 0.f);
-    float4 dk[NS], dv[NS], dc[NS], cvn[NS], wc[NS], w3v[NS];
+    float4 dk[NS], dv_[NS], dc[NS], cvn[NS], wc[NS], w3v[NS];
 #pragma unroll
     for (int s = 0; s < NS; ++s) {
         const int c = s * 256 + lane * 4;
-        dk[s] = z4; dv[s] = z4; dc[s] = z4; cvn[s] = z4; wc[s] = z4; w3v[s] = z4;
+        dk[s] = z4; dv_[s] = z4; dc[s] = z4; cvn[s] = z4; wc[s] = z4; w3v[s] = z4;
         if (c < H && idx < n_act) {
             cvn[s] = *(const float4*)(cv + (size_t)n * ldcv + c);
             wc[s] = *(const float4*)(wcr + c); w3v[s] = *(const float4*)(w3 + c);
@@ -487,7 +494,7 @@
                         const float4 qm = *(const float4*)(qkv + (size_t)m * ldqkv + c);
                         const float4 gm = *(const float4*)(dh_out + (size_t)m * H + c);
                         dk[s].x += dl * qm.x; dk[s].y += dl * qm.y; dk[s].z += dl * qm.z; dk[s].w += dl * qm.w;
-                        dv[s].x += al * gm.x; dv[s].y += al * gm.y; dv[s].z += al * gm.z; dv[s].w += al * gm.w;
+                        dv_[s].x += al * gm.x; dv_[s].y += al * gm.y; dv_[s].z += al * gm.z; dv_[s].w += al * gm.w;
                         dc[s].x += dcm * w3v[s].x * dsilu_f(cvn[s].x + rh * wc[s].x);
                         dc[s].y += dcm * w3v[s].y * dsilu_f(cvn[s].y + rh * wc[s].y);
                         dc[s].z += dcm * w3v[s].z * dsilu_f(cvn[s].z + rh * wc[s].z);
@@ -502,9 +509,9 @@
         for (int s = 0; s < NS; ++s) {
             const int c = s * 256 + lane * 4;
             if (c < H) {
-                *(float4*)(dqkv + (size_t)n * ldqkv + H + c) = dk[s];
-                *(float4*)(dqkv + (size_t)n * ldqkv + 2 * H + c) = dv[s];
-                *(float4*)(dcv + (size_t)n * ldcv + c) = dc[s];
+                st_grad4<O16>(dqkv, (size_t)n * ldo + H + c, dk[s]);
+                *(float4*)(dv + (size_t)n * lddv + c) = dv_[s];
+                st_grad4<O16>(dcv, (size_t)n * ldoc + c, dc[s]);
             }
         }
         return;
@@ -512,7 +519,7 @@
 #pragma unroll
     for (int s = 0; s < NS; ++s) {
         shb[(0 * 4 + wv) * NS * 64 + s * 64 + lane] = dk[s];
-        shb[(1 * 4 + wv) * NS * 64 + s * 64 + lane] = dv[s];
+        shb[(1 * 4 + wv) * NS * 64 + s * 64 + lane] = dv_[s];
         shb[(2 * 4 + wv) * NS * 64 + s * 64 + lane] = dc[s];
     }
     __syncthreads();
@@ -526,10 +533,34 @@
             const float4 o = shb[(qn * 4 + w) * NS * 64 + g];
             t.x += o.x; t.y += o.y; t.z += o.z; t.w += o.w;
         }
-        if (qn == 0) *(float4*)(dqkv + (size_t)n * ldqkv + H + c) = t;
-        else if (qn == 1) *(float4*)(dqkv + (size_t)n * ldqkv + 2 * H + c) = t;
-        else *(float4*)(dcv + (size_t)n * ldcv + c) = t;
-    }
+        if (qn == 0) st_grad4<O16>(dqkv, (size_t)n * ldo + H + c, t);
+        else if (qn == 1) *(float4*)(dv + (size_t)n * lddv + c) = t;
+        else st_grad4<O16>(dcv, (size_t)n * ldoc + c, t);
+    }
+}
+
+template <bool O16>
+static int inter_attn_bwd_rows_launch(const float* qkv, int ldqkv, const float* cv, int ldcv, int H, const float* d, const float* rhohat,
+                                      const int* rowptr, const int* col, const int* mirror, const int* red_idx, const float* w_rk,
+                                      const float* w_rv, const float* wcr, const float* w3, const float* alpha, const float* cvs,
+                                      float clampv, int n_rows, const float* dh_out, const float* dx_out, void* dqkv, int ldo, float* dv,
+                                      int lddv, void* dcv, int ldoc, float* dd, float* drh, float* dbias_red, float* dlogit, float* dcp,
+                                      float* wpart, int nblk, const int* order, int n_heavy, int n_act, hipStream_t stream) {
+    dim3 gb(n_heavy + (n_rows - n_heavy + 3) / 4);
+#define LA(NS) do {                                                                                                    \
+        size_t lds = (size_t)16 * NS * 64 * sizeof(float4);                                                            \
+        hipLaunchKernelGGL((inter_attn_bwd_a_rows_kernel<NS, O16>), dim3(nblk), dim3(256), lds, stream, qkv, ldqkv, cv, ldcv, H, d, \
+                           rhohat, rowptr, col, w_rk, w_rv, wcr, w3, alpha, cvs, clampv, n_rows, dh_out, dx_out, dqkv, ldo, dd, \
+                           drh, dlogit, dcp, wpart, order, n_heavy, n_act);                                             \
+        size_t ldsb = (size_t)12 * NS * 64 * sizeof(float4);                                                           \
+        hipLaunchKernelGGL((inter_attn_bwd_b_rows_kernel<NS, O16>), gb, dim3(256), ldsb, stream, qkv, ldqkv, cv, ldcv, H, rhohat, rowptr, \
+                           col, mirror, red_idx, wcr, w3, alpha, dlogit, dcp, n_rows, dh_out, dqkv, ldo, dv, lddv, dcv, ldoc,  \
+                           dbias_red, order, n_heavy, n_act);                                                          \
+    } while (0)
+    if (H <= 256) LA(1); else if (H <= 512) LA(2); else LA(4);
+#undef LA
+    FB_CHECK_LAUNCH();
+    return 0;
 }
 
 extern "C" int fabind_inter_attn_bwd_rows(const float* qkv, int ldqkv, const float* cv, int ldcv, int H, const float* d,
@@ -542,19 +573,27 @@
     if (n_rows <= 0) return 0;
     FB_REQUIRE(H % 4 == 0 && H <= 1024, "fabind_inter_attn_bwd_rows: H % 4, H <= 1024");
     FB_REQUIRE(order != nullptr && 0 <= n_heavy && n_heavy <= n_act && n_act <= n_rows && nblk > 0, "fabind_inter_attn_bwd_rows: order / counts");
-    dim3 gb(n_heavy + (n_rows - n_heavy + 3) / 4);
-#define LA(NS) do {                                                                                                    \
-        size_t lds = (size_t)16 * NS * 64 * sizeof(float4);                                                            \
-        hipLaunchKernelGGL((inter_attn_bwd_a_rows_kernel<NS>), dim3(nblk), dim3(256), lds, stream, qkv, ldqkv, cv, ldcv, H, d, \
-                           rhohat, rowptr, col, w_rk, w_rv, wcr, w3, alpha, cvs, clampv, n_rows, dh_out, dx_out, dqkv, dd, \
-                           drh, dlogit, dcp, wpart, order, n_heavy, n_act);                                             \
-        size_t ldsb = (size_t)12 * NS * 64 * sizeof(float4);                                                           \
-        hipLaunchKernelGGL((inter_attn_bwd_b_rows_kernel<NS>), gb, dim3(256), ldsb, stream, qkv, ldqkv, cv, ldcv, H, rhohat, rowptr, \
-                           col, mirror, red_idx, wcr, w3, alpha, dlogit, dcp, n_rows, dh_out, dqkv, dcv, dbias_red, order,  \
-                           n_heavy, n_act);                                                                            \
-    } while (0)
-    if (H <= 256) LA(1); else if (H <= 512) LA(2); else LA(4);
-#undef LA
-    FB_CHECK_LAUNCH();
-    return 0;
-}
+    return inter_attn_bwd_rows_launch<false>(qkv, ldqkv, cv, ldcv, H, d, rhohat, rowptr, col, mirror, red_idx, w_rk, w_rv, wcr, w3, alpha, cvs,
+                                             clampv, n_rows, dh_out, dx_out, dqkv, ldqkv, dqkv + 2 * H, ldqkv, dcv, ldcv, dd, drh, dbias_red,
+                                             dlogit, dcp, wpart, nblk, order, n_heavy, n_act, stream);
+}
+
+extern "C" int fabind_inter_attn_bwd_rows_b16(const float* qkv, int ldqkv, const float* cv, int ldcv, int H, const float* d,
+                                              const float* rhohat, const int* rowptr, const int* col, const int* mirror,
+                                              const int* red_idx, const float* w_rk, const float* w_rv, const float* wcr,
+                                              const float* w3, const float* alpha, const float* cvs, float clampv, int n_rows,
+                                              const float* dh_out, const float* dx_out, void* dqk16, int ldo, float* dv32, int lddv,
+                                              void* dcv16, int ldoc, float* dd, float* drh, float* dbias_red, float* dlogit,
+                                              float* dcp, float* wpart, int nblk, const int* order, int n_heavy, int n_act,
+                                              hipStream_t stream) {
+    if (n_rows <= 0) return 0;
+    FB_REQUIRE(H % 4 == 0 && H <= 1024, "fabind_inter_attn_bwd_rows_b16: H % 4, H <= 1024");
+    FB_REQUIRE(order != nullptr && 0 <= n_heavy && n_heavy <= n_act && n_act <= n_rows && nblk > 0, "fabind_inter_attn_bwd_rows_b16: order / counts");
+    FB_REQUIRE(dqk16 != nullptr && dv32 != nullptr && dcv16 != nullptr && ldo >= 2 * H && lddv >= H && ldoc >= H,
+               "fabind_inter_attn_bwd_rows_b16: outputs / leading dimensions");
+    FB_REQUIRE(ldo % 4 == 0 && ldoc % 4 == 0 && lddv % 4 == 0 && ((uintptr_t)dqk16 & 7) == 0 && ((uintptr_t)dcv16 & 7) == 0 && ((uintptr_t)dv32 & 15) == 0,
+               "fabind_inter_attn_bwd_rows_b16: ldo / ldoc / lddv % 4 == 0, 8-byte aligned bf16 outputs, 16-byte aligned dv32");
+    return inter_attn_bwd_rows_launch<true>(qkv, ldqkv, cv, ldcv, H, d, rhohat, rowptr, col, mirror, red_idx, w_rk, w_rv, wcr, w3, alpha, cvs,
+                                            clampv, n_rows, dh_out, dx_out, dqk16, ldo, dv32, lddv, dcv16, ldoc, dd, drh, dbias_red,
+                                            dlogit, dcp, wpart, nblk, order, n_heavy, n_act, stream);
+}
diff --git a/fabind_amd/engine.py b/fabind_amd/engine.py
--- a/fabind_amd/engine.py
+++ b/fabind_amd/engine.py
@@ -585,10 +585,10 @@
     ab32 = ops.linear(h16, p["W_ab32"], p["b_ab32"])
     hd = ops.pair_hadamard(a0b0, H, ab32, 64, g.red_p, g.red_c, graph=g)
     bias_part = ops.linear_rowdot(hd, p["Wcomp1"], p["bcomp1"], p["u"], act_epi=K.ACT_RELU)
-    qkv = ops.linear(h if p.get("Wqkv32") is not None else h16, p["Wqkv"], p["bqkv"], want16=True, W32=p.get("Wqkv32"))
+    qkv_lin = (h if p.get("Wqkv32") is not None else h16, p["Wqkv"], p["bqkv"], p.get("Wqkv32"))
     d, rhohat = ops.edge_geom(x, g.row_int, g.col_int, g.rp_int, lay, g.int_by_col)
-    h_new, x_new, alpha = ops.inter_attn(qkv, None, H, h, x, d, rhohat, g, bias_part, p["w_rk"], p["w_rv"], p["wcr"],
-                                         p["w3"], clampv, Wc=p["Wc"], bc=p["bc"], own_h=(pdrop == 0.0), Wc32=p.get("Wc32"))
+    h_new, x_new, alpha = ops.inter_attn(None, None, H, h, x, d, rhohat, g, bias_part, p["w_rk"], p["w_rv"], p["wcr"],
+                                         p["w3"], clampv, Wc=p["Wc"], bc=p["bc"], own_h=(pdrop == 0.0), Wc32=p.get("Wc32"), qkv_lin=qkv_lin)
     if pdrop > 0.0:
         h_new = ops.drop_mix(h, h_new, pdrop)
     return h_new, x_new, alpha
diff --git a/fabind_amd/kernels.py b/fabind_amd/kernels.py
--- a/fabind_amd/kernels.py
+++ b/fabind_amd/kernels.py
@@ -47,7 +47,7 @@
 def gemm(A, W, bias=None, A2=None, act_pro=ACT_NONE, act_epi=ACT_NONE, residual=None, r_index=None,
          out=None, out_dtype=torch.float32, want_out=True, dotvec=None, aux=None, dact=ACT_NONE, alpha=1.0,
          accumulate=False, groups=None, n_groups=0, max_m=0, max_n=0, M=None, N=None, ldc=None, k_splits=1,
-         out2=None, groups_ext=False, p_drop=0.0, seed=0, out16=None, flops=None, force_x3=False):
+         out2=None, groups_ext=False, p_drop=0.0, seed=0, out16=None, flops=None, force_x3=False, plan_only=False):
     lib = _lib.load()
     a = GemmArgs()
     K1 = A.shape[1]
@@ -91,6 +91,10 @@
     a.p_drop, a.drop_seed = float(p_drop), int(seed) & 0xFFFFFFFF
     x3 = A.dtype == torch.float32 and W.dtype == torch.float32 and (_split3() or force_x3)
     a.split3 = 1 if x3 else 0
+    if plan_only:
+        fam, epi, cfg = ctypes.c_int(-9), ctypes.c_int(-9), ctypes.c_int(-9)
+        check(lib.fabind_gemm_plan(ctypes.byref(a), ctypes.byref(fam), ctypes.byref(epi), ctypes.byref(cfg)), "fabind_gemm_plan")
+        return fam.value, epi.value, cfg.value
     if PROFILE is None:
         check(lib.fabind_gemm(ctypes.byref(a), stream()), "fabind_gemm")
         return (out if want_out else None), dot_out
diff --git a/fabind_amd/ops.py b/fabind_amd/ops.py
--- a/fabind_amd/ops.py
+++ b/fabind_amd/ops.py
@@ -181,6 +181,10 @@
         return dpre, (db if with_db else None)
     if kind == "none":
         return dy, None
+    if kind == "cast" and md == torch.bfloat16:
+        c = getattr(dy, "_fab_b16", None)
+        if c is not None and c[0] == dy._version and c[1].shape == dy.shape:
+            return c[1], None
     scale = scale if kind == "act" else 1.0
     return _mul_dact_colsum(dy, aux, act, md, scale) if with_db else (_mul_dact(dy, aux, act, md, scale), None)
 
@@ -220,6 +224,12 @@
 def _attach_b16(y, y16):
     if y16 is not None:
         y._fab_b16 = (y._version, y16)
+    return y
+
+
+def _dy16_hint(y, on):
+    if on and y.dtype == torch.float32 and mm_dtype() == torch.bfloat16:
+        y._fab_dy16 = True
     return y
 
 
@@ -335,7 +345,7 @@
         K.tn_hook(W, b)
         holder = [] if _want16(out_dtype, act_epi, want16) else None
         y = _Linear.apply(x, W, b, x2, residual, act_epi, out_dtype, holder, p_drop, seed, W32)
-        return _attach_b16(y, holder[0] if holder else None)
+        return _attach_b16(_dy16_hint(y, act_epi == K.ACT_NONE and p_drop == 0.0), holder[0] if holder else None)
     y16 = None
     if _want16(out_dtype, act_epi, want16) and act_pro == K.ACT_NONE and (p_drop == 0.0 or (act_epi == K.ACT_NONE and x2 is None and W.shape[0] % 4 == 0)):
         y16 = torch.empty((x.shape[0], W.shape[0]), dtype=torch.bfloat16, device=x.device)
@@ -428,7 +438,7 @@
         K.tn_hook(W1, b1, W2, b2)
         holder = [] if _want16(torch.float32, K.ACT_NONE, want16) else None
         y = _MLP2.apply(x, x2, W1, b1, W2, b2, residual, act, holder, p_drop, _drop_seed(p_drop), W32, chain if W32 is not None else None)
-        return _attach_b16(y, holder[0] if holder else None)
+        return _attach_b16(_dy16_hint(y, p_drop == 0.0), holder[0] if holder else None)
     if W32 is not None:
         t = linear(x, W1, b1, act_epi=act, x2=x2, out_dtype=torch.float32, W32=W32[0])
         return linear(t, W2, b2, residual=residual, want16=want16, W32=W32[1])
@@ -937,8 +947,13 @@
         idx, = ctx.saved_tensors
         d_rows = dout.index_select(0, idx)
         if dout.is_contiguous() and _owned_grad(dout):
+            c = getattr(dout, "_fab_b16", None)
+            keep = c is not None and c[0] == dout._version
             d_base = dout
             d_base.index_fill_(0, idx, 0.0)
+            if keep:
+                c[1].index_fill_(0, idx, 0.0)
+                d_base._fab_b16 = (d_base._version, c[1])
         else:
             d_base = dout.index_fill(0, idx, 0.0)
         return d_base, d_rows, None, None
@@ -962,6 +977,8 @@
         c = getattr(base, "_fab_b16", None)
         keep = c is not None and c[0] == base._version
         out = _PutRows.apply(base, rows, index64, inplace)
+        if getattr(base, "_fab_dy16", False):
+            out._fab_dy16 = True
         if keep and inplace:
             out._fab_b16 = (out._version, c[1])
         return out
@@ -982,6 +999,7 @@
         self.pending = None
         self.rows = []
         self.deferred = []
+        self.want16 = False
 
     def take(self, like):
         if self.buf is None:
@@ -1038,7 +1056,7 @@
 DEFER_DX_MIN_ROWS = 1024
 
 
-def _run_deferred(defs, out, base, accumulate):
+def _run_deferred(defs, out, base, accumulate, out16=None):
     defs = sorted(defs, key=lambda d_: -d_[0].shape[1])
     first = True
     while defs:
@@ -1050,6 +1068,8 @@
         else:
             (A1, Wcat), = defs
             defs, args = [], {}
+        if not defs and out16 is not None:
+            args["out16"] = out16
         if first and not accumulate:
             K.gemm(A1, Wcat, out=out, residual=base, **args)
         else:
@@ -1071,9 +1091,12 @@
         pend, rows, defs = sink.pending, sink.rows, sink.deferred
         owned = g is not None and g is sink.buf
         sink.buf, sink.pending, sink.rows, sink.deferred = None, None, [], []
+        g16 = None
+        if defs and sink.want16 and ctx.meta[1] == torch.float32 and mm_dtype() == torch.bfloat16 and ctx.meta[0][-1] % 4 == 0:
+            g16 = torch.empty(ctx.meta[0], dtype=torch.bfloat16, device=ctx.meta[2])
         if defs:
             if owned:
-                _run_deferred(defs, g, None, True)
+                _run_deferred(defs, g, None, True, g16)
             else:
                 base = g
                 if pend is not None:
@@ -1081,7 +1104,7 @@
                 if base is not None and base.dtype != ctx.meta[1] and not (base.dtype == torch.bfloat16 and ctx.meta[1] == torch.float32):
                     base = base.to(ctx.meta[1])
                 g = torch.empty(ctx.meta[0], dtype=ctx.meta[1], device=ctx.meta[2])
-                _run_deferred(defs, g, base, False)
+                _run_deferred(defs, g, base, False, g16)
                 owned = True
         if pend is not None:
             if g is None:
@@ -1096,8 +1119,13 @@
             owned = True
             for idx, r in rows:
                 g.index_add_(0, idx, r.to(g.dtype))
+            if g16 is not None:
+                for idx, _ in rows:
+                    g16.index_copy_(0, idx, g.index_select(0, idx).to(torch.bfloat16))
         if owned:
             g._fab_owned = True
+        if g16 is not None:
+            g._fab_b16 = (g._version, g16)
         return g, None
 
 
@@ -1105,6 +1133,7 @@
     if not (torch.is_grad_enabled() and t.requires_grad):
         return t
     sink = GradSink()
+    sink.want16 = bool(getattr(t, "_fab_dy16", False))
     out = _SinkOwner.apply(t, sink)
     out._fab_gsink = sink
     c = getattr(t, "_fab_b16", None)
@@ -1299,8 +1328,15 @@
 
 class _InterAttn(torch.autograd.Function):
     @staticmethod
-    def forward(ctx, qkv, cv, h, x, d, rhohat, bias_part, w_rk, w_rv, wcr, w3, H, g, clampv, s_ext=None, Wc=None, bc=None, holder=None, Wc32=None):
-        v_in = None
+    def forward(ctx, qkv, cv, h, x, d, rhohat, bias_part, w_rk, w_rv, wcr, w3, H, g, clampv, s_ext=None, Wc=None, bc=None, holder=None, Wc32=None,
+                xq=None, Wq=None, bq=None, Wq32=None):
+        v_in = xq_in = None
+        if Wq is not None:
+            xq_in = _mm_in(xq)
+            qkv = torch.empty((xq.shape[0], Wq.shape[0]), dtype=torch.float32, device=xq.device)
+            q16 = torch.empty(qkv.shape, dtype=torch.bfloat16, device=xq.device) if _want16(torch.float32, K.ACT_NONE, True) else None
+            _linear_fwd(xq, xq_in, None, None, Wq, Wq32, bq, qkv, y16=q16)
+            _attach_b16(qkv, q16)
         if Wc is not None:
             c16 = getattr(qkv, "_fab_b16", None) if _cfg.get_precision() == "bf16" else None
             v_in = c16[1][:, 2 * H:] if (c16 is not None and c16[0] == qkv._version) else _mm_in(qkv[:, 2 * H:])
@@ -1315,23 +1351,34 @@
         h_out, x_out, alpha, cvs = K.inter_attn_fwd(qkv, cv, H, h, x, d, rhohat, g.rp_int, g.col_int, g.red_idx,
                                                     bias_part, w_rk, w_rv, wcr, w3, clampv, s_ext, h16, deal=getattr(g, "int_deal", None))
         ctx.g, ctx.H, ctx.clampv, ctx.np = g, H, clampv, bias_part.shape[1]
-        ctx.has_ext, ctx.has_cv = s_ext is not None, Wc is not None
+        ctx.has_ext, ctx.has_cv, ctx.has_q = s_ext is not None, Wc is not None, Wq is not None
         ctx.sink_h, ctx.Wct = _sink_of(h), (_stored_wt(Wc) if Wc is not None else None)
-        ctx.save_for_backward(qkv, cv, d, rhohat, w_rk, w_rv, wcr, w3, alpha, cvs, v_in, Wc)
+        ctx.sink_xq, ctx.Wqt = _sink_of(xq), (_stored_wt(Wq) if Wq is not None else None)
+        ctx.xq_dtype, ctx.has_bq = (xq.dtype if xq is not None else None), bq is not None
+        ctx.save_for_backward(qkv, cv, d, rhohat, w_rk, w_rv, wcr, w3, alpha, cvs, v_in, Wc, xq_in, Wq)
         ctx.mark_non_differentiable(alpha)
         return h_out, x_out, alpha
 
     @staticmethod
     def backward(ctx, dh_out, dx_out, _dalpha):
-        qkv, cv, d, rhohat, w_rk, w_rv, wcr, w3, alpha, cvs, v_in, Wc = ctx.saved_tensors
+        qkv, cv, d, rhohat, w_rk, w_rv, wcr, w3, alpha, cvs, v_in, Wc, xq_in, Wq = ctx.saved_tensors
         g, H = ctx.g, ctx.H
         N, E = qkv.shape[0], g.col_int.shape[0]
         dev = qkv.device
         f32 = dict(dtype=torch.float32, device=dev)
+        ni = ctx.needs_input_grad
         dh_out = dh_out.contiguous() if dh_out is not None else torch.zeros((N, H), **f32)
         dx_out = dx_out.contiguous() if dx_out is not None else torch.zeros((N, 3), **f32)
-        dqkv = torch.empty_like(qkv)
-        dcv = torch.empty_like(cv)
+        deal = getattr(g, "int_deal", None) if K.INTER_ATTN_ROWS else None
+        out16 = (ctx.has_q and ctx.has_cv and deal is not None and mm_dtype() == torch.bfloat16 and H % 8 == 0
+                 and Wc.dtype == torch.bfloat16 and Wq.dtype == torch.bfloat16)
+        if out16:
+            dqkv = torch.empty((N, 3 * H), dtype=torch.bfloat16, device=dev)
+            dv32 = torch.empty((N, H), **f32)
+            dcv = torch.empty((N, H), dtype=torch.bfloat16, device=dev)
+        else:
+            dqkv = torch.empty_like(qkv)
+            dcv = torch.empty_like(cv)
         dd, drh = torch.empty((max(E, 1), 3), **f32), torch.empty(max(E, 1), **f32)
         n_red = E // 2
         dbias_red = torch.zeros(max(n_red, 1), **f32)
@@ -1340,8 +1387,14 @@
             dd.zero_(); drh.zero_()
         nblk = min((N + 3) // 4, INTER_BWD_BLOCKS)
         wpart = torch.empty((nblk, 4 * H), **f32)
-        deal = getattr(g, "int_deal", None) if K.INTER_ATTN_ROWS else None
-        if deal is not None:
+        if out16:
+            check(load().fabind_inter_attn_bwd_rows_b16(ptr(qkv), qkv.stride(0), ptr(cv), cv.stride(0), H, ptr(d), ptr(rhohat),
+                                                        ptr(g.rp_int), ptr(g.col_int), ptr(g.mirror), ptr(g.red_idx), ptr(w_rk),
+                                                        ptr(w_rv), ptr(wcr), ptr(w3), ptr(alpha), ptr(cvs), ctx.clampv, N, ptr(dh_out),
+                                                        ptr(dx_out), ptr(dqkv), 3 * H, ptr(dv32), H, ptr(dcv), H, ptr(dd), ptr(drh),
+                                                        ptr(dbias_red), ptr(dlogit), ptr(dcp), ptr(wpart), nblk, ptr(deal[0]),
+                                                        int(deal[1]), int(deal[2]), stream()), "fabind_inter_attn_bwd_rows_b16")
+        elif deal is not None:
             check(load().fabind_inter_attn_bwd_rows(ptr(qkv), qkv.stride(0), ptr(cv), cv.stride(0), H, ptr(d), ptr(rhohat),
                                                     ptr(g.rp_int), ptr(g.col_int), ptr(g.mirror), ptr(g.red_idx), ptr(w_rk),
                                                     ptr(w_rv), ptr(wcr), ptr(w3), ptr(alpha), ptr(cvs), ctx.clampv, N, ptr(dh_out),
@@ -1358,30 +1411,60 @@
         dw = [dw_all[i * H:(i + 1) * H] for i in range(4)]
         dWc = dbc = None
         if ctx.has_cv:
-            ni = ctx.needs_input_grad
             dpre, dbc = _dpre(dcv, K.ACT_NONE, None, 1.0, None, ni[16], ni[15])
-            K.gemm(dpre, _wt(ctx.Wct, Wc), out=dqkv[:, 2 * H:], accumulate=True)
+            if out16:
+                K.gemm(dpre, _wt(ctx.Wct, Wc), out=dv32, accumulate=True, out16=dqkv[:, 2 * H:])
+                del dv32
+            else:
+                K.gemm(dpre, _wt(ctx.Wct, Wc), out=dqkv[:, 2 * H:], accumulate=True)
             dWc, dbc = _param_grads(dpre, v_in, None, Wc, ni[15], ni[16], dbc)
             dcv = None
         if ctx.sink_h is not None and ctx.needs_input_grad[2]:
             dh_out = ctx.sink_h.deposit(dh_out)
+        dxq = dWq = dbq = None
+        if ctx.has_q:
+            want_dW, want_db = ni[20], ctx.has_bq and ni[21]
+            dpre, dbq = _dpre(dqkv, K.ACT_NONE, None, 1.0, None, want_db, want_dW)
+            if ni[19]:
+                dmm, Wt = _padded_k(dpre, Wq, ctx.Wqt, (Wq.shape[0] + 7) // 8 * 8)
+                sink_x = ctx.sink_xq if ctx.xq_dtype in (torch.float32, torch.bfloat16) else None
+                if sink_x is not None:
+                    dxq = sink_x.gemm_into(dmm, Wt, xq_in, ctx.xq_dtype)
+                else:
+                    dxq, _ = K.gemm(dmm, Wt, out_dtype=torch.float32 if ctx.xq_dtype == torch.float32 else ctx.xq_dtype)
+            dWq, dbq = _param_grads(dpre, xq_in, None, Wq, want_dW, want_db, dbq)
+            dqkv = None
         return (dqkv, dcv, dh_out, dx_out, dd[:E], drh[:E], dbias_red[:n_red, None].expand(n_red, ctx.np), dw[0], dw[1],
-                dw[2], dw[3], None, None, None, dcp[:E] if ctx.has_ext else None, dWc, dbc, None, None)
+                dw[2], dw[3], None, None, None, dcp[:E] if ctx.has_ext else None, dWc, dbc, None, None, dxq, dWq, dbq, None)
 
 
 INTER_BWD_BLOCKS = 1024
 
 
-def inter_attn(qkv, cv, H, h, x, d, rhohat, g, bias_part, w_rk, w_rv, wcr, w3, clampv, s_ext=None, Wc=None, bc=None, own_h=False, Wc32=None):
+def inter_attn(qkv, cv, H, h, x, d, rhohat, g, bias_part, w_rk, w_rv, wcr, w3, clampv, s_ext=None, Wc=None, bc=None, own_h=False, Wc32=None,
+               qkv_lin=None):
     assert (cv is None) != (Wc is None), "inter_attn: pass either cv or its Linear (Wc, bc)"
+    assert (qkv is None) != (qkv_lin is None), "inter_attn: pass either qkv or its Linear (xq, Wqkv, bqkv, Wqkv32)"
+    xq = Wq = bq = Wq32 = None
+    if qkv_lin is not None:
+        xq, Wq, bq, Wq32 = qkv_lin
+        if not (_needs_grad(xq, Wq, bq, cv, h, x, d, rhohat, bias_part, w_rk, w_rv, wcr, w3, s_ext, Wc, bc) and Wc is not None
+                and mm_dtype() == torch.bfloat16 and xq.dim() == 2 and xq.stride(-1) == 1 and Wq.shape[0] == 3 * H):
+            qkv, xq, Wq, bq, Wq32 = linear(xq, Wq, bq, want16=True, W32=Wq32), None, None, None, None
+        elif not _split_site_ok(xq, Wq, Wq32, None, K.ACT_NONE, torch.float32, 0.0):
+            Wq32 = None
     w16 = _cfg.get_precision() == "bf16" and h.is_contiguous()
-    if Wc32 is not None and not (Wc is not None and _cfg.get_precision() == "bf16" and qkv.dtype == torch.float32 and Wc32.dtype == torch.float32
-                                 and tuple(Wc32.shape) == tuple(Wc.shape) and qkv.stride(0) % 4 == 0):
+    q_f32, q_ld = (qkv.dtype == torch.float32, qkv.stride(0)) if qkv is not None else (True, 3 * H)
+    if Wc32 is not None and not (Wc is not None and _cfg.get_precision() == "bf16" and q_f32 and Wc32.dtype == torch.float32
+                                 and tuple(Wc32.shape) == tuple(Wc.shape) and q_ld % 4 == 0):
         Wc32 = None
-    if _needs_grad(qkv, cv, h, x, d, rhohat, bias_part, w_rk, w_rv, wcr, w3, s_ext, Wc, bc):
+    if _needs_grad(qkv, cv, h, x, d, rhohat, bias_part, w_rk, w_rv, wcr, w3, s_ext, Wc, bc, xq, Wq, bq):
         K.tn_hook(Wc, bc)
+        if Wq is not None:
+            K.tn_hook(Wq, bq)
         holder = [] if w16 else None
-        h_out, x_out, alpha = _InterAttn.apply(qkv, cv, h, x, d, rhohat, bias_part, w_rk, w_rv, wcr, w3, H, g, clampv, s_ext, Wc, bc, holder, Wc32)
+        h_out, x_out, alpha = _InterAttn.apply(qkv, cv, h, x, d, rhohat, bias_part, w_rk, w_rv, wcr, w3, H, g, clampv, s_ext, Wc, bc, holder, Wc32,
+                                               xq, Wq, bq, Wq32)
         return _attach_b16(h_out, holder[0] if holder else None), x_out, alpha
     if cv is None:
         cv = linear(qkv[:, 2 * H:], Wc, bc, W32=Wc32)
diff --git a/include/fabind_hip.h b/include/fabind_hip.h
--- a/include/fabind_hip.h
+++ b/include/fabind_hip.h
@@ -451,6 +451,13 @@
                                const float* cvs, float clampv, int n_rows, const float* dh_out, const float* dx_out,
                                float* dqkv, float* dcv, float* dd, float* drh, float* dbias_red, float* dlogit, float* dcp,
                                float* wpart, int nblk, const int* order, int n_heavy, int n_act, hipStream_t stream);
+int fabind_inter_attn_bwd_rows_b16(const float* qkv, int ldqkv, const float* cv, int ldcv, int H, const float* d,
+                                   const float* rhohat, const int* rowptr, const int* col, const int* mirror, const int* red_idx,
+                                   const float* w_rk, const float* w_rv, const float* wcr, const float* w3, const float* alpha,
+                                   const float* cvs, float clampv, int n_rows, const float* dh_out, const float* dx_out,
+                                   void* dqk16, int ldo, float* dv32, int lddv, void* dcv16, int ldoc, float* dd, float* drh,
+                                   float* dbias_red, float* dlogit, float* dcp, float* wpart, int nblk, const int* order,
+                                   int n_heavy, int n_act, hipStream_t stream);
 int fabind_las_step_bwd(const float* x, const float* x0, const unsigned char* pass_mask, const int* las_i, const int* las_j,
                         const int* las_off, const int* node_off, const int* c_cnt, int B, int max_n, float step,
                         float clampv, const float* dout, float* dx, hipStream_t stream);
```

After: 528.3. 1.6% lower.
